# unirestore/UniRestore

Hardware: AMD Instinct MI355X
Metric: restored 512x512 images/sec @ 20 denoise steps (whole job) (higher is better)
Workload: dtype bf16; 1 GPU; PIR 512x512 batch=8/GPU, 20 DDIM steps, bf16, hipGraph replay (BASELINE.json configs[1]; configs[2] shape for N=8); global_batch=8, per_gpu_batch=8, image=512, denoise_steps=20, parallelism=image-parallel dp1, weights=seeded random init (no checkpoints reachable)

## Files before the change

### include/unirestore_hip.h

```cpp
#ifndef UNIRESTORE_HIP_H
#define UNIRESTORE_HIP_H

#include <stddef.h>
#include <stdint.h>

#ifdef __cplusplus
extern "C" {
#endif

typedef void* ur_stream_t;

enum { UR_OK = 0, UR_E_INVALID = -1, UR_E_UNSUPPORTED = -2, UR_E_LAUNCH = -3, UR_E_WORKSPACE = -4 };

enum { UR_DT_BF16 = 0, UR_DT_F16 = 1 };

enum {
  UR_ACT_NONE = 0,
  UR_ACT_SILU = 1,
  UR_ACT_GELU = 2,
  UR_ACT_GEGLU = 3,
  UR_ACT_GATE = 4,
  UR_ACT_TANH = 5,
  UR_ACT_RELU = 6
};

int ur_version(void);
const char* ur_last_error(void);

typedef struct ur_conv_desc {
  const void* x;
  const void* x2;
  const void* w;
  const float* bias;
  const void* residual;
  void* y;
  void* yt;
  float* gn_part;
  const float* gn_ab;
  int gn_silu;
  float* row_stats;
  const float* ln_stats;
  const float* ln_colsum;
  float ln_eps;
  int ln_dim;
  int ln_parts;
  float* workspace;
  size_t workspace_bytes;
  int N, H, W;
  int C1, ldx, C2, ldx2;
  int Cout, ldw, ldy, ldr;
  int KH, KW, stride, pad_t, pad_l;
  int OH, OW;
  int upsample2x;
  int act;
  int out_f32;
  int n_split, t_rows, t_ld;
  float out_scale;
  int nbatch;
  long long bs_x, bs_x2, bs_w, bs_bias, bs_y, bs_r;
  int k_chunk_major;
  long long bias_img_stride;
  int dtype;
  const void* w_frag;
} ur_conv_desc;

int ur_conv2d_nhwc(const ur_conv_desc* d, ur_stream_t stream);

typedef struct ur_conv_plan {
  int row_stat_parts;
  int gn_parts;
  int gn_fused;
  int prologue_ok;
} ur_conv_plan;
int ur_conv2d_plan(const ur_conv_desc* d, ur_conv_plan* plan);

typedef struct ur_conv_launch_info {
  int launcher;
  int splitk;
  int nk_per_split;
  int reduce;
  int reduce_ri;
  int gn_pass;
  int group_loop;
} ur_conv_launch_info;
int ur_conv2d_plan_launch(const ur_conv_desc* d, ur_conv_launch_info* info);
int ur_conv_launcher_count(void);
const char* ur_conv_launcher_name(int i);

int ur_gemm_bias_act(const void* x, const void* w, const float* bias, const void* residual, void* y, long long M, int N, int K,
                     int ldx, int ldw, int ldy, int ldr, int act, float* workspace, size_t workspace_bytes, int dtype,
                     ur_stream_t stream);
int ur_groupconv3x3_nhwc(const void* x, const void* w, const float* bias, void* y, int N, int H, int W, int Cg, int Cog,
                         int groups, int act, float* workspace, size_t workspace_bytes, int dtype, ur_stream_t stream);

int ur_groupnorm_stats_parts(int N, int HW, int C);
size_t ur_groupnorm_ws_bytes(int N, int HW, int C);
size_t ur_groupnorm_ab_bytes(int N, int C);
int ur_groupnorm_stats(const void* x, float* part, int N, int HW, int C, int dtype, ur_stream_t stream);
int ur_instnorm_stats(const void* x, float* part, int N, int HW, int C, int dtype, ur_stream_t stream);
int ur_groupnorm_finalize(const float* part1, int parts1, int C1, const float* part2, int parts2, int C2, const float* gamma,
                          const float* beta, int N, int HW, int G, float eps, float* ab, float* mean_out, ur_stream_t stream);
int ur_groupnorm_apply_act(const void* x, const void* x2, void* y, const float* ab, int N, int HW, int C1, int C2, int silu,
                           int dtype, ur_stream_t stream);
int ur_groupnorm_nhwc(const void* x, const void* x2, void* y, const float* gamma, const float* beta, int N, int HW,
                      int C1, int C2, int G, float eps, int silu, float* ws, float* ab, const float* pre1, int parts1,
                      const float* pre2, int parts2, int dtype, ur_stream_t stream);
int ur_layernorm_rows(const void* x, void* y, const float* gamma, const float* beta, long long rows, int C,
                      float eps, int dtype, ur_stream_t stream);
int ur_softmax_rows_f32(const float* s, void* p, long long rows, int cols, int ldp, int dtype, ur_stream_t stream);

int ur_attention_fwd(const void* q, const void* k, const void* vt, void* o, int B, int H, int Tq, int Tk,
                     int D, int ldq, int ldk, int ldvt, int ldo, long long bs_q, long long bs_k,
                     long long bs_vt, long long bs_o, float scale, int dtype, ur_stream_t stream);
size_t ur_attention_workspace_bytes(int B, int H, int Tq, int Tk, int D);
int ur_attention_fwd_ws(const void* q, const void* k, const void* vt, void* o, int B, int H, int Tq, int Tk,
                        int D, int ldq, int ldk, int ldvt, int ldo, long long bs_q, long long bs_k, long long bs_vt,
                        long long bs_o, float scale, void* ws, size_t ws_bytes, int dtype, ur_stream_t stream);
typedef struct ur_attention_plan {
  int kernel;
  int workgroups;
  int n_full;
  int n_split;
} ur_attention_plan;
int ur_attention_plan_launch(const void* q, const void* k, const void* vt, void* o, int B, int H, int Tq, int Tk,
                             int D, int ldq, int ldk, int ldvt, int ldo, long long bs_q, long long bs_k, long long bs_vt,
                             long long bs_o, void* ws, size_t ws_bytes, ur_attention_plan* plan);
int ur_attention_kernel_count(void);
const char* ur_attention_kernel_name(int i);

size_t ur_chain_tile_bytes(void);
int ur_ff_geglu_fused(const void* x, const void* stream_w, size_t stream_bytes, void* y, long long T, int C, int hidden, int ldx,
                      int ldy, float ln_eps, int dtype, ur_stream_t stream);

int ur_transformer_head_fused(const void* x, const float* gn_ab, const void* stream_w, size_t stream_bytes, void* h0, void* q, void* k,
                              void* vt, long long T, int tokens_per_image, int C, float ln_eps, int dtype, ur_stream_t stream);
int ur_transformer_tail_fused(const void* o1, const void* h0, const void* xres, const void* stream_w, size_t stream_bytes, void* y,
                              float* gn_part, long long T, int tokens_per_image, int C, int hidden, int heads, int tk, float ln_eps,
                              float attn_scale, int dtype, ur_stream_t stream);

int ur_csce_fused(const void* x, const void* cond, const void* stream_w, size_t stream_bytes, void* y, float* gn_part, long long T,
                  int tokens_per_image, int C, int Ccond, int dtype, ur_stream_t stream);

int ur_dwconv3x3_nhwc(const void* x, const float* w9c, const float* bias, void* y, int N, int H, int W, int C,
                      int gate, int dtype, ur_stream_t stream);
int ur_avgpool_hw(const void* x, float* out, int N, int HW, int C, float* ws, int dtype, ur_stream_t stream);
int ur_scale_channels(const void* x, const float* s, const void* residual, void* y, int N, int HW, int C,
                      int dtype, ur_stream_t stream);
int ur_axpy_channels(const void* a, const void* b, const float* s, void* y, long long rows, int C, int dtype, ur_stream_t stream);
int ur_spade_modulate(const void* n, const void* gb, int ldgb, const void* residual, void* y, long long rows, int C,
                      int dtype, ur_stream_t stream);
int ur_linear_f32(const float* x, const float* w, const float* bias, float* y, int M, int N, int K, int groups,
                  int act, ur_stream_t stream);
int ur_tfa_prompt_update(const float* pooled, const float* cond, float* upd, int B, int T, int D, ur_stream_t stream);
int ur_scale_channels_fanout(const void* x, const float* s, void* y, int B, int K, int HW, int C, int dtype, ur_stream_t stream);
int ur_tfa_prompt_update_fanout(const float* pooled, const float* cond, float* upd, int B, int K, int T, int D, int cond_per_row,
                                ur_stream_t stream);
int ur_vec_mul_group(const float* a, const float* b, float* out, int N, int C, int G, ur_stream_t stream);

int ur_image_to_nhwc(const float* img, void* y, int N, int C, int H, int W, int Cpad, int dtype, ur_stream_t stream);
int ur_nhwc_to_nchw_f32(const void* x, int x_is_f32, float* out, int N, int C, int H, int W, int ld, float mul,
                        float add, int dtype, ur_stream_t stream);
int ur_nchw_f32_to_nhwc(const float* x, void* y, int N, int C, int H, int W, int Cpad, int dtype, ur_stream_t stream);
int ur_image_resize_pad_nhwc(const float* img, void* y, int N, int C, int H, int W, int RH, int RW, int PH, int PW, int Cpad,
                             float mul, float add, int dtype, ur_stream_t stream);
int ur_image_unpad_resize_nchw(const void* x, int x_is_f32, float* out, int N, int C, int XH, int XW, int ld, int CH, int CW,
                               int OH, int OW, float mul, float add, int quantize, int dtype, ur_stream_t stream);
int ur_image_u8_ingest(const uint8_t* src, long long slot_bytes, const int* geom, void* y, int N, int CH, int CW, int Cpad, float mul,
                       float add, int dtype, ur_stream_t stream);
int ur_image_u8_egress(const void* x, int x_is_f32, uint8_t* dst, long long slot_bytes, const int* geom, int* nonfinite, int N, int C,
                       int XH, int XW, int ld, float mul, float add, int dtype, ur_stream_t stream);
int ur_vae_sample(const float* moments, int ld, const float* noise_nchw, float* z_nhwc, void* z_16, int N,
                  int HW, int Clat, int Cpad, float scale, int dtype, ur_stream_t stream);
int ur_add_noise(const float* z0, const float* noise_nchw, float* zt, void* zt_16, int N, int HW, int Clat,
                 int Cpad, float sa, float sb, int dtype, ur_stream_t stream);
int ur_ddim_step(float* zt, const float* eps, int ld_eps, void* zt_16, long long M, int Clat, int Cpad,
                 float c_x, float c_e, int dtype, ur_stream_t stream);
int ur_latent_tiles_gather(const float* z, void* tiles_16, int N, int LH, int LW, int Cpad, int T, int th, int tw,
                           const int* origins, int dtype, ur_stream_t stream);
int ur_latent_tiles_blend_ddim(float* zt, const float* eps_tiles, int ld_eps, void* zt_tiles_16, const float* wn, int N, int LH,
                               int LW, int Clat, int Cpad, int T, int th, int tw, const int* origins, float c_x, float c_e,
                               int dtype, ur_stream_t stream);
int ur_f32_to_bf16_scaled(const float* x, int ld, void* y, long long M, int C, int Cpad, float mul, int dtype, ur_stream_t stream);

int ur_keyed_noise(const uint32_t* keys, uint32_t draw, void* out, int N, long long count, int kind, ur_stream_t stream);

int ur_image_metrics(const float* pred, const float* target, int N, int C, int H, int W, int win, double data_range,
                     double* psnr, double* ssim, void* ws, long long ws_bytes, ur_stream_t stream);
long long ur_image_metrics_ws_size(int N, int C, int H, int W, int win);

int ur_lpips_prep(const float* x, float* y, int N, int C, int H, int W, ur_stream_t stream);
int ur_conv2d_f32_wpack_dims(int Cin, int Cout, int KH, int KW, int* kpad, int* cout_pad);
int ur_conv2d_f32(const float* x, const float* w, const float* bias, float* y, int N, int H, int W, int Cin, int Cout, int KH, int KW,
                  int stride, int pad, int relu, ur_stream_t stream);
int ur_maxpool2d_f32(const float* x, float* y, int N, int H, int W, int C, ur_stream_t stream);
int ur_lpips_tap_hw(int H, int W, int tap, int* oh, int* ow);
long long ur_lpips_layer_parts(long long P);
int ur_lpips_layer(const float* feat, const float* lin, int N, int P, int C, double* part, long long part_bytes, ur_stream_t stream);
long long ur_lpips_ws_size(int N, int H, int W);
int ur_lpips_finish(const void* ws, long long ws_bytes, int N, int H, int W, double* out, ur_stream_t stream);

int ur_conv2d_f32_res(const float* x, const float* w, const float* bias, const float* res, float* y, int N, int H, int W, int Cin, int Cout,
                      int KH, int KW, int stride, int pad, int relu, ur_stream_t stream);
int ur_classify_preprocess(const float* x, float* tmp, float* y, int N, int C, int H, int W, const int* first_w, const int* count_w,
                           const float* wt_w, int taps_w, const int* first_h, const int* count_h, const float* wt_h, int taps_h,
                           ur_stream_t stream);
int ur_maxpool2d_pad_f32(const float* x, float* y, int N, int H, int W, int C, ur_stream_t stream);
int ur_avgpool_f32(const float* x, float* y, int N, int P, int C, ur_stream_t stream);
int ur_top1_counts(const float* logits, const long long* labels, int N, int C, long long* pred, long long* counts, ur_stream_t stream);

int ur_color_fix_wavelet(const void* c_f32, int ld_c, const void* src_16, int ld_s, float* out, int N, int src_n, int H, int W, int dtype,
                         ur_stream_t stream);
int ur_color_fix_adain(const void* c_f32, int ld_c, const void* src_16, int ld_s, float* out, int N, int src_n, int H, int W, int dtype,
                       void* ws, size_t ws_bytes, ur_stream_t stream);
size_t ur_color_fix_adain_ws_bytes(int N, int H, int W);

int ur_corrupt_noise(const uint8_t* x, const uint32_t* keys, void* out, int N, int H, int W, int mode, float c, const uint32_t* table,
                     int out_kind, ur_stream_t stream);
int ur_corrupt_filter_sep(const uint8_t* x, const float* taps, int radius, void* out, int N, int H, int W, void* ws, size_t ws_bytes,
                          int out_kind, ur_stream_t stream);
size_t ur_corrupt_filter_sep_ws_bytes(int N, int H, int W);
int ur_corrupt_taps(const uint8_t* x, const int32_t* taps, int n_taps, int per_image, int border, void* out, int N, int H, int W,
                    int out_kind, ur_stream_t stream);
int ur_corrupt_zoom(const uint8_t* x, const int32_t* layers, int n_layers, void* out, int N, int H, int W, int out_kind, ur_stream_t stream);
int ur_corrupt_color(const uint8_t* x, void* out, int N, int H, int W, int mode, float a, float b, void* ws, size_t ws_bytes, int out_kind,
                     ur_stream_t stream);
size_t ur_corrupt_color_ws_bytes(int N, int H, int W);
int ur_corrupt_pixelate(const uint8_t* x, void* out, int N, int H, int W, int small_h, int small_w, const int32_t* hbox, const int32_t* vbox,
                        const int32_t* ymap, const int32_t* xmap, void* ws, size_t ws_bytes, int out_kind, ur_stream_t stream);
size_t ur_corrupt_pixelate_ws_bytes(int N, int H, int small_w);
int ur_corrupt_fog(const uint8_t* x, const uint32_t* keys, void* out, int N, int H, int W, float c, double decay, void* ws, size_t ws_bytes,
                   int out_kind, ur_stream_t stream);
size_t ur_corrupt_fog_ws_bytes(int N, int H, int W);

int ur_jpeg_roundtrip(const uint8_t* x, uint8_t* out, int N, int H, int W, int quality, int subsampling, void* ws, size_t ws_bytes,
                      ur_stream_t stream);
size_t ur_jpeg_roundtrip_ws_bytes(int N, int H, int W, int subsampling);

int ur_resize_u8(const uint8_t* x, uint8_t* out, int N, int H, int W, int oh, int ow, const int32_t* xbounds, const int32_t* xweights, int xK,
                 int xp, const int32_t* ybounds, const int32_t* yweights, int yK, int yp, void* ws, size_t ws_bytes, ur_stream_t stream);
size_t ur_resize_u8_ws_bytes(int N, int H, int W, int oh, int ow);

int ur_distort_shuffle(const uint8_t* x, const uint32_t* keys, uint8_t* out, int N, int H, int W, int delta, uint32_t draw, ur_stream_t stream);
int ur_distort_snow_layer(const uint32_t* keys, float* field, int N, int H, int W, int top, int left, int ch, int cw, int oh, int ow, float loc,
                          float scale, float thr, ur_stream_t stream);
int ur_distort_snow(const uint8_t* x, const float* field, const int32_t* taps, int n_taps, void* out, int N, int H, int W, int oh, int ow,
                    float keep, void* ws, size_t ws_bytes, int out_kind, ur_stream_t stream);
size_t ur_distort_snow_ws_bytes(int N, int H, int W);
int ur_distort_field(const uint32_t* keys, const float* taps_y, int ry, const float* taps_x, int rx, float* field, int N, int H, int W, float m,
                     float alpha, void* ws, size_t ws_bytes, ur_stream_t stream);
size_t ur_distort_field_ws_bytes(int N, int H, int W);
int ur_distort_warp(const uint8_t* x, const float* field, void* out, int N, int H, int W, int out_kind, ur_stream_t stream);

int ur_profile_enable(int on);
int ur_profile_report(char* buf, size_t buf_bytes);

#ifdef __cplusplus
// ... 4 lines not shown
```

### unirestore_amd/capi.py

```python
import ctypes as C
import os

import torch

_HERE = os.path.dirname(os.path.abspath(__file__))
LIB_PATH = os.environ.get("UR_LIB") or os.path.join(_HERE, "libunirestore_hip.so")

UR_ACT_NONE, UR_ACT_SILU, UR_ACT_GELU, UR_ACT_GEGLU, UR_ACT_GATE, UR_ACT_TANH, UR_ACT_RELU = range(7)
UR_DT_BF16, UR_DT_F16 = 0, 1
UR_E_INVALID, UR_E_UNSUPPORTED = -1, -2


class ConvDesc(C.Structure):
    _fields_ = [
        ("x", C.c_void_p), ("x2", C.c_void_p), ("w", C.c_void_p), ("bias", C.c_void_p), ("residual", C.c_void_p),
        ("y", C.c_void_p), ("yt", C.c_void_p), ("gn_part", C.c_void_p), ("gn_ab", C.c_void_p), ("gn_silu", C.c_int),
        ("row_stats", C.c_void_p), ("ln_stats", C.c_void_p), ("ln_colsum", C.c_void_p), ("ln_eps", C.c_float), ("ln_dim", C.c_int), ("ln_parts", C.c_int),
        ("workspace", C.c_void_p),
        ("workspace_bytes", C.c_size_t),
        ("N", C.c_int), ("H", C.c_int), ("W", C.c_int),
        ("C1", C.c_int), ("ldx", C.c_int), ("C2", C.c_int), ("ldx2", C.c_int),
        ("Cout", C.c_int), ("ldw", C.c_int), ("ldy", C.c_int), ("ldr", C.c_int),
        ("KH", C.c_int), ("KW", C.c_int), ("stride", C.c_int), ("pad_t", C.c_int), ("pad_l", C.c_int),
        ("OH", C.c_int), ("OW", C.c_int),
        ("upsample2x", C.c_int), ("act", C.c_int), ("out_f32", C.c_int),
        ("n_split", C.c_int), ("t_rows", C.c_int), ("t_ld", C.c_int),
        ("out_scale", C.c_float),
        ("nbatch", C.c_int),
        ("bs_x", C.c_longlong), ("bs_x2", C.c_longlong), ("bs_w", C.c_longlong), ("bs_bias", C.c_longlong),
        ("bs_y", C.c_longlong), ("bs_r", C.c_longlong), ("k_chunk_major", C.c_int), ("bias_img_stride", C.c_longlong),
        ("dtype", C.c_int), ("w_frag", C.c_void_p),
    ]


class ConvPlan(C.Structure):
    _fields_ = [("row_stat_parts", C.c_int), ("gn_parts", C.c_int), ("gn_fused", C.c_int), ("prologue_ok", C.c_int)]


class ConvLaunchInfo(C.Structure):
    _fields_ = [("launcher", C.c_int), ("splitk", C.c_int), ("nk_per_split", C.c_int), ("reduce", C.c_int), ("reduce_ri", C.c_int),
                ("gn_pass", C.c_int), ("group_loop", C.c_int)]


class AttentionPlan(C.Structure):
    _fields_ = [("kernel", C.c_int), ("workgroups", C.c_int), ("n_full", C.c_int), ("n_split", C.c_int)]


_P, _I, _F, _LL, _SZ = C.c_void_p, C.c_int, C.c_float, C.c_longlong, C.c_size_t

SIGNATURES = {
    "ur_version": (_I, []),
    "ur_last_error": (C.c_char_p, []),
    "ur_conv2d_nhwc": (_I, [C.POINTER(ConvDesc), _P]),
    "ur_conv2d_plan": (_I, [C.POINTER(ConvDesc), C.POINTER(ConvPlan)]),
    "ur_conv2d_plan_launch": (_I, [C.POINTER(ConvDesc), C.POINTER(ConvLaunchInfo)]),
    "ur_conv_launcher_count": (_I, []),
    "ur_conv_launcher_name": (C.c_char_p, [_I]),
    "ur_gemm_bias_act": (_I, [_P, _P, _P, _P, _P, _LL, _I, _I, _I, _I, _I, _I, _I, _P, _SZ, _I, _P]),
    "ur_groupconv3x3_nhwc": (_I, [_P, _P, _P, _P, _I, _I, _I, _I, _I, _I, _I, _P, _SZ, _I, _P]),
    "ur_groupnorm_stats_parts": (_I, [_I, _I, _I]),
    "ur_groupnorm_ws_bytes": (_SZ, [_I, _I, _I]),
    "ur_groupnorm_ab_bytes": (_SZ, [_I, _I]),
    "ur_groupnorm_stats": (_I, [_P, _P, _I, _I, _I, _I, _P]),
    "ur_instnorm_stats": (_I, [_P, _P, _I, _I, _I, _I, _P]),
    "ur_groupnorm_finalize": (_I, [_P, _I, _I, _P, _I, _I, _P, _P, _I, _I, _I, _F, _P, _P, _P]),
    "ur_groupnorm_apply_act": (_I, [_P, _P, _P, _P, _I, _I, _I, _I, _I, _I, _P]),
    "ur_groupnorm_nhwc": (_I, [_P, _P, _P, _P, _P, _I, _I, _I, _I, _I, _F, _I, _P, _P, _P, _I, _P, _I, _I, _P]),
    "ur_layernorm_rows": (_I, [_P, _P, _P, _P, _LL, _I, _F, _I, _P]),
    "ur_softmax_rows_f32": (_I, [_P, _P, _LL, _I, _I, _I, _P]),
    "ur_attention_fwd": (_I, [_P, _P, _P, _P, _I, _I, _I, _I, _I, _I, _I, _I, _I, _LL, _LL, _LL, _LL, _F, _I, _P]),
    "ur_attention_workspace_bytes": (_SZ, [_I, _I, _I, _I, _I]),
    "ur_attention_fwd_ws": (_I, [_P, _P, _P, _P, _I, _I, _I, _I, _I, _I, _I, _I, _I, _LL, _LL, _LL, _LL, _F, _P, _SZ, _I, _P]),
    "ur_attention_plan_launch": (_I, [_P, _P, _P, _P, _I, _I, _I, _I, _I, _I, _I, _I, _I, _LL, _LL, _LL, _LL, _P, _SZ, C.POINTER(AttentionPlan)]),
    "ur_attention_kernel_count": (_I, []),
    "ur_attention_kernel_name": (C.c_char_p, [_I]),
    "ur_chain_tile_bytes": (_SZ, []),
    "ur_ff_geglu_fused": (_I, [_P, _P, _SZ, _P, _LL, _I, _I, _I, _I, _F, _I, _P]),
    "ur_transformer_head_fused": (_I, [_P, _P, _P, _SZ, _P, _P, _P, _P, _LL, _I, _I, _F, _I, _P]),
    "ur_transformer_tail_fused": (_I, [_P, _P, _P, _P, _SZ, _P, _P, _LL, _I, _I, _I, _I, _I, _F, _F, _I, _P]),
    "ur_csce_fused": (_I, [_P, _P, _P, _SZ, _P, _P, _LL, _I, _I, _I, _I, _P]),
    "ur_dwconv3x3_nhwc": (_I, [_P, _P, _P, _P, _I, _I, _I, _I, _I, _I, _P]),
    "ur_avgpool_hw": (_I, [_P, _P, _I, _I, _I, _P, _I, _P]),
    "ur_scale_channels": (_I, [_P, _P, _P, _P, _I, _I, _I, _I, _P]),
    "ur_scale_channels_fanout": (_I, [_P, _P, _P, _I, _I, _I, _I, _I, _P]),
    "ur_axpy_channels": (_I, [_P, _P, _P, _P, _LL, _I, _I, _P]),
    "ur_spade_modulate": (_I, [_P, _P, _I, _P, _P, _LL, _I, _I, _P]),
    "ur_linear_f32": (_I, [_P, _P, _P, _P, _I, _I, _I, _I, _I, _P]),
    "ur_tfa_prompt_update": (_I, [_P, _P, _P, _I, _I, _I, _P]),
    "ur_tfa_prompt_update_fanout": (_I, [_P, _P, _P, _I, _I, _I, _I, _I, _P]),
    "ur_vec_mul_group": (_I, [_P, _P, _P, _I, _I, _I, _P]),
    "ur_image_to_nhwc": (_I, [_P, _P, _I, _I, _I, _I, _I, _I, _P]),
    "ur_nhwc_to_nchw_f32": (_I, [_P, _I, _P, _I, _I, _I, _I, _I, _F, _F, _I, _P]),
    "ur_nchw_f32_to_nhwc": (_I, [_P, _P, _I, _I, _I, _I, _I, _I, _P]),
    "ur_image_resize_pad_nhwc": (_I, [_P, _P] + [_I] * 9 + [_F, _F, _I, _P]),
    "ur_image_unpad_resize_nchw": (_I, [_P, _I, _P] + [_I] * 9 + [_F, _F, _I, _I, _P]),
    "ur_image_u8_ingest": (_I, [_P, _LL, _P, _P, _I, _I, _I, _I, _F, _F, _I, _P]),
    "ur_image_u8_egress": (_I, [_P, _I, _P, _LL, _P, _P, _I, _I, _I, _I, _I, _F, _F, _I, _P]),
    "ur_vae_sample": (_I, [_P, _I, _P, _P, _P, _I, _I, _I, _I, _F, _I, _P]),
    "ur_add_noise": (_I, [_P, _P, _P, _P, _I, _I, _I, _I, _F, _F, _I, _P]),
    "ur_ddim_step": (_I, [_P, _P, _I, _P, _LL, _I, _I, _F, _F, _I, _P]),
    "ur_latent_tiles_gather": (_I, [_P, _P, _I, _I, _I, _I, _I, _I, _I, _P, _I, _P]),
    "ur_latent_tiles_blend_ddim": (_I, [_P, _P, _I, _P, _P, _I, _I, _I, _I, _I, _I, _I, _I, _P, _F, _F, _I, _P]),
    "ur_f32_to_bf16_scaled": (_I, [_P, _I, _P, _LL, _I, _I, _F, _I, _P]),
    "ur_keyed_noise": (_I, [_P, C.c_uint32, _P, _I, _LL, _I, _P]),
    "ur_image_metrics": (_I, [_P, _P, _I, _I, _I, _I, _I, C.c_double, _P, _P, _P, _LL, _P]),
    "ur_image_metrics_ws_size": (_LL, [_I, _I, _I, _I, _I]),
    "ur_lpips_prep": (_I, [_P, _P, _I, _I, _I, _I, _P]),
    "ur_conv2d_f32_wpack_dims": (_I, [_I, _I, _I, _I, C.POINTER(_I), C.POINTER(_I)]),
    "ur_conv2d_f32": (_I, [_P, _P, _P, _P] + [_I] * 10 + [_P]),
    "ur_maxpool2d_f32": (_I, [_P, _P, _I, _I, _I, _I, _P]),
    "ur_lpips_tap_hw": (_I, [_I, _I, _I, C.POINTER(_I), C.POINTER(_I)]),
    "ur_lpips_layer_parts": (_LL, [_LL]),
    "ur_lpips_layer": (_I, [_P, _P, _I, _I, _I, _P, _LL, _P]),
    "ur_lpips_ws_size": (_LL, [_I, _I, _I]),
    "ur_lpips_finish": (_I, [_P, _LL, _I, _I, _I, _P, _P]),
    "ur_conv2d_f32_res": (_I, [_P, _P, _P, _P, _P] + [_I] * 10 + [_P]),
    "ur_classify_preprocess": (_I, [_P, _P, _P, _I, _I, _I, _I, _P, _P, _P, _I, _P, _P, _P, _I, _P]),
    "ur_maxpool2d_pad_f32": (_I, [_P, _P, _I, _I, _I, _I, _P]),
    "ur_avgpool_f32": (_I, [_P, _P, _I, _I, _I, _P]),
    "ur_top1_counts": (_I, [_P, _P, _I, _I, _P, _P, _P]),
    "ur_color_fix_wavelet": (_I, [_P, _I, _P, _I, _P, _I, _I, _I, _I, _I, _P]),
    "ur_color_fix_adain": (_I, [_P, _I, _P, _I, _P, _I, _I, _I, _I, _I, _P, _SZ, _P]),
    "ur_color_fix_adain_ws_bytes": (_SZ, [_I, _I, _I]),
    "ur_corrupt_noise": (_I, [_P, _P, _P, _I, _I, _I, _I, _F, _P, _I, _P]),
    "ur_corrupt_filter_sep": (_I, [_P, _P, _I, _P, _I, _I, _I, _P, _SZ, _I, _P]),
    "ur_corrupt_filter_sep_ws_bytes": (_SZ, [_I, _I, _I]),
    "ur_corrupt_taps": (_I, [_P, _P, _I, _I, _I, _P, _I, _I, _I, _I, _P]),
    "ur_corrupt_zoom": (_I, [_P, _P, _I, _P, _I, _I, _I, _I, _P]),
    "ur_corrupt_color": (_I, [_P, _P, _I, _I, _I, _I, _F, _F, _P, _SZ, _I, _P]),
    "ur_corrupt_color_ws_bytes": (_SZ, [_I, _I, _I]),
    "ur_corrupt_pixelate": (_I, [_P, _P, _I, _I, _I, _I, _I, _P, _P, _P, _P, _P, _SZ, _I, _P]),
    "ur_corrupt_pixelate_ws_bytes": (_SZ, [_I, _I, _I]),
    "ur_corrupt_fog": (_I, [_P, _P, _P, _I, _I, _I, _F, C.c_double, _P, _SZ, _I, _P]),
    "ur_corrupt_fog_ws_bytes": (_SZ, [_I, _I, _I]),
    "ur_jpeg_roundtrip": (_I, [_P, _P, _I, _I, _I, _I, _I, _P, _SZ, _P]),
    "ur_jpeg_roundtrip_ws_bytes": (_SZ, [_I, _I, _I, _I]),
    "ur_resize_u8": (_I, [_P, _P, _I, _I, _I, _I, _I, _P, _P, _I, _I, _P, _P, _I, _I, _P, _SZ, _P]),
    "ur_resize_u8_ws_bytes": (_SZ, [_I, _I, _I, _I, _I]),
    "ur_distort_shuffle": (_I, [_P, _P, _P, _I, _I, _I, _I, C.c_uint32, _P]),
    "ur_distort_snow_layer": (_I, [_P, _P, _I, _I, _I, _I, _I, _I, _I, _I, _I, _F, _F, _F, _P]),
    "ur_distort_snow": (_I, [_P, _P, _P, _I, _P, _I, _I, _I, _I, _I, _F, _P, _SZ, _I, _P]),
    "ur_distort_snow_ws_bytes": (_SZ, [_I, _I, _I]),
    "ur_distort_field": (_I, [_P, _P, _I, _P, _I, _P, _I, _I, _I, _F, _F, _P, _SZ, _P]),
    "ur_distort_field_ws_bytes": (_SZ, [_I, _I, _I]),
    "ur_distort_warp": (_I, [_P, _P, _P, _I, _I, _I, _I, _P]),
    "ur_profile_enable": (_I, [_I]),
    "ur_profile_report": (_I, [C.c_char_p, _SZ]),
}


def _load():
    if not os.path.exists(LIB_PATH):
        raise ImportError(
            f"{LIB_PATH} not found: build it with `python -m unirestore_amd.build` (or __graft_entry__.build()). "
            "There is no CPU / eager fallback in the product path.")
    lib = C.CDLL(LIB_PATH)
    for name, (res, args) in SIGNATURES.items():
        fn = getattr(lib, name)
        fn.restype, fn.argtypes = res, args
    return lib


lib = _load()


def launcher_names() -> list:
    return [lib.ur_conv_launcher_name(i).decode() for i in range(lib.ur_conv_launcher_count())]


def plan_launch(d: ConvDesc) -> ConvLaunchInfo:
    info = ConvLaunchInfo()
    check(lib.ur_conv2d_plan_launch(d, info))
    return info


def attention_kernel_names() -> list:
    return [lib.ur_attention_kernel_name(i).decode() for i in range(lib.ur_attention_kernel_count())]


def attention_plan(q, k, vt, o, B, H, Tq, Tk, D, ldq, ldk, ldvt, ldo, bs_q, bs_k, bs_vt, bs_o, ws, ws_bytes) -> AttentionPlan:
    plan = AttentionPlan()
    check(lib.ur_attention_plan_launch(q, k, vt, o, B, H, Tq, Tk, D, ldq, ldk, ldvt, ldo, bs_q, bs_k, bs_vt, bs_o, ws, ws_bytes, plan))
    return plan


class URError(RuntimeError):
    pass


def check(rc: int):
    if rc != 0:
        msg = lib.ur_last_error().decode("utf-8", "replace")
        if rc == UR_E_INVALID:
            raise ValueError(f"unirestore_hip: {msg}")
        if rc == UR_E_UNSUPPORTED:
            raise NotImplementedError(f"unirestore_hip (UR_E_UNSUPPORTED): {msg}")
        raise URError(f"unirestore_hip error {rc}: {msg}")
```

### unirestore_amd/csrc/igemm.hip

```cpp
#include "igemm_impl.h"

namespace urk {
#define UR_DECLARE(name)                                                                                             \
  ConvLaunch name##_bf16(void* k, size_t ws_bytes);                                                                 \
  ConvLaunch name##_f16(void* k, size_t ws_bytes);                                                                  \
  static ConvLaunch name(ConvK& k, size_t ws_bytes) { return (k.f16 ? name##_f16 : name##_bf16)(&k, ws_bytes); }
UR_CONV_LAUNCHERS(UR_DECLARE)
#undef UR_DECLARE
}

namespace {

ConvLaunch dispatch_conv(ConvK& k, bool pair, size_t ws_bytes) {
  if (k.KH == 3 && k.stride == 1 && k.pad_t == 1 && k.pad_l == 1 && k.kcm && k.staged_ok_ && !pair && k.nbatch == 1 &&
      k.OW % 32 == 0 && k.OH % 8 == 0 && k.OH == (k.ups ? 2 * k.H : k.H) && k.OW == (k.ups ? 2 * k.W : k.W) && !k.yt) {
    const bool ok128 = k.Cout % 128 == 0, ok160 = k.Cout % 160 == 0;
    const long long tm8 = (long long)k.N * (k.OH / 8) * (k.OW / 32);
    auto eff = [](long long t) { return t <= 128 ? (double)(t * (256 / t)) / 256.0 : (double)t / (double)(((t + 255) / 256) * 256); };
    const bool use160 = ok160 && (!ok128 || eff(tm8 * (k.Cout / 160)) >= eff(tm8 * (k.Cout / 128)));
    const long long tiles8 = tm8 * (use160 ? k.Cout / 160 : k.Cout / 128);
    if ((ok128 || ok160) && tiles8 >= 64) {
      if (use160) return urk::halo_8x32_160(k, ws_bytes);
      return urk::halo_8x32_128(k, ws_bytes);
    }
  }
  if (k.KH == 3 && k.stride == 1 && k.pad_t == 1 && k.pad_l == 1 && k.kcm && !pair && k.nbatch == 1 && !k.ups && k.C2 == 0 &&
      k.Cout <= 32 && k.OW % 32 == 0 && k.OH % 8 == 0 && k.OH == k.H && k.OW == k.W && !k.yt && !k.gn_part && !k.gn_ab && !k.row_stats && !k.ln_stats &&
      !k.bias_img && (long long)k.N * (k.OH / 8) * (k.OW / 32) >= 128)
    return urk::halo_thin_32(k, ws_bytes);
  const bool himg_ups = k.ups && k.OH == 16 && k.OW == 16 && k.H == 8 && k.W == 8;
  if (k.KH == 3 && k.stride == 1 && k.pad_t == 1 && k.pad_l == 1 && k.kcm && k.staged_ok_ && !pair && k.nbatch == 1 &&
      ((!k.ups && k.OH == k.H && k.OW == k.W) || himg_ups) && !k.yt && k.Cout % 128 == 0 && k.nk >= 36) {
    if (k.wf && k.OH == 8 && k.OW == 8 && k.N <= 16 && k.Cin % 256 == 0 && k.nk >= 72 && k.y && k.ws && !k.gn_ab && !k.row_stats && !k.ln_stats &&
        (long long)(k.nk / 36) * k.M * k.Cout * 4 <= (long long)ws_bytes)
      return urk::wstream_8x8(k, ws_bytes);
    if (k.OH == 16 && k.OW == 16) return urk::himg_16x16(k, ws_bytes);
    if (k.OH == 8 && k.OW == 8 && k.N % 4 == 0) {
      return urk::himg_8x8x4(k, ws_bytes);
    }
  }
  if (k.KH == 1 && k.stride == 1 && !k.ups && k.C2 == 0 && k.staged_ok_ && k.Cout % 256 == 0 && !k.yt && (k.act == UR_ACT_GEGLU || k.act == UR_ACT_GATE) &&
      (long long)((k.M + 255) / 256) * (k.Cout / 256) * k.nbatch >= 200 && (long long)k.M * k.ldx < (1ll << 31) - 256)
  {
    auto fill = [](long long t) { return (double)t / (double)(((t + 255) / 256) * 256); };
    const long long tm = (k.M + 255) / 256;
    if (k.Cout % 320 == 0 && k.nbatch == 1 && !k.bias_img && fill(tm * (k.Cout / 320)) > fill(tm * (k.Cout / 256)))
      return urk::gemm_256x320_pair(k, ws_bytes);
    return urk::gemm_256x256(k, ws_bytes);
  }
  const bool use_v1 = k.KH == 1 && k.nk <= 10;
  const long long blocks128 = (long long)((k.M + 127) / 128) * ((k.Cout + 127) / 128) * k.nbatch;
  const bool g1 = k.KH == 1 && k.stride == 1 && !k.ups && k.C2 == 0 && k.pad_t == 0 && k.pad_l == 0 && k.OH == k.H && k.OW == k.W &&
                  (long long)k.M * k.ldx + k.Ktot < (1ll << 31) - 256;
  auto nosplit = [&](int bm, int bn) { return (long long)((k.M + bm - 1) / bm) * ((k.Cout + bn - 1) / bn) * k.nbatch >= 200 || k.nk < 8 || !k.ws; };
  if (k.KH == 1 && !pair && k.Cout > 64) {
    const long long blocks64 = (long long)((k.M + 63) / 64) * ((k.Cout + 63) / 64) * k.nbatch;
    if (blocks128 < 200 && g1 && blocks64 >= 128 && blocks64 <= 256 && k.nk >= 8 && k.nk <= 48) return urk::g1_64x64_deep(k, ws_bytes);
    if (g1 && blocks128 < 200 && k.nk > 24 && k.nk <= 96 && (long long)((k.M + 127) / 128) * ((k.Cout + 63) / 64) * k.nbatch >= 256)
      return urk::g1_128x64_deep(k, ws_bytes);
    if (blocks128 < 200 && g1 && ((blocks64 >= 128 && k.nk <= 24) || (blocks64 >= 256 && k.nk <= 48))) return urk::g1_64x64(k, ws_bytes);
    if (blocks128 < 200 && k.nk <= 24) return g1 && nosplit(64, 64) ? urk::g1_64x64(k, ws_bytes) : urk::v1_64x64(k, ws_bytes);
    if (use_v1 && blocks128 > 256 && blocks128 < 400 && k.Cout % 128 == 0) return g1 && nosplit(128, 64) ? urk::g1_128x64(k, ws_bytes) : urk::v1_128x64(k, ws_bytes);
  }
  if (use_v1) {
    if (pair) return urk::v1_128x128(k, ws_bytes);
    if (k.Cout <= 32) return urk::v1_256x32(k, ws_bytes);
    if (k.Cout <= 64) return urk::v1_128x64(k, ws_bytes);
    if (k.Cout % 160 == 0 && k.Cout % 128 != 0) return g1 && nosplit(128, 160) ? urk::g1_128x160(k, ws_bytes) : urk::v1_128x160(k, ws_bytes);
    return g1 && nosplit(128, 128) ? urk::g1_128x128(k, ws_bytes) : urk::v1_128x128(k, ws_bytes);
  }
  if (k.Cout <= 32) return urk::v2_256x32(k, ws_bytes);
  if (k.Cout <= 64 && !pair) return urk::v2_128x64(k, ws_bytes);
  const bool n160 = !pair && k.Cout % 160 == 0 && k.Cout % 128 != 0;
  const long long big_tiles = (long long)((k.M + 255) / 256) * ((k.Cout + (n160 ? 159 : 127)) / (n160 ? 160 : 128)) * k.nbatch;
  if (g1 && !pair && big_tiles < 256) {
    const long long t160 = k.Cout % 160 == 0 ? (long long)((k.M + 127) / 128) * (k.Cout / 160) : 0;
    const long long t128 = (long long)((k.M + 127) / 128) * ((k.Cout + 127) / 128);
    auto fill = [](long long t) { return t <= 0 ? 0.0 : (double)t / (double)(((t + 255) / 256) * 256); };
    if (t160 >= 200 && fill(t160) >= fill(t128)) return urk::g1_128x160(k, ws_bytes);
    if (t128 >= 200) return urk::g1_128x128(k, ws_bytes);
  }
  if (big_tiles >= 160) {
    if (n160 && g1) return urk::g1_128x160(k, ws_bytes);
    if (n160) return urk::v2_256x160(k, ws_bytes);
    return urk::v2_256x128(k, ws_bytes);
  }
  if (k.Cout % 160 == 0 && k.Cout % 128 != 0 && !pair) return urk::v1_128x160(k, ws_bytes);
  return urk::v1_128x128(k, ws_bytes);
}

}

static int conv_impl(const ur_conv_desc* d, ur_stream_t stream, ur_conv_plan* plan, ur_conv_launch_info* info = nullptr) {
  UR_REQUIRE(d && d->x && d->w, "null x/w");
  UR_REQUIRE(d->KH == d->KW && (d->KH == 1 || d->KH == 3), "only 1x1 and 3x3 kernels");
  UR_REQUIRE(d->C1 > 0 && d->C1 % 8 == 0 && d->C2 % 8 == 0 && d->ldx % 8 == 0, "Cin/ldx must be multiples of 8");
  UR_REQUIRE(d->C2 == 0 || (d->x2 && d->ldx2 % 8 == 0), "virtual concat needs x2");
  UR_REQUIRE(d->Cout > 0 && d->Cout % 4 == 0 && d->ldw % 8 == 0, "Cout%4, ldw%8");
  UR_REQUIRE(d->nbatch >= 1 && d->stride >= 1 && d->OH > 0 && d->OW > 0, "bad dims");
  UR_REQUIRE(d->y || d->yt || d->gn_part, "no output requested");
  UR_REQUIRE_DT(d->dtype);
  const bool pair = d->act == UR_ACT_GEGLU || d->act == UR_ACT_GATE;
  if (pair && d->Cout % 64 != 0)
    return ur::fail(UR_E_UNSUPPORTED, "ur_conv2d_nhwc: pair activations (GEGLU / SimpleGate) need Cout % 64 == 0 (32-row a|g interleave)");
  UR_REQUIRE(!d->y || (d->out_f32 ? d->ldy % 4 == 0 : d->ldy % 4 == 0), "ldy%4");
  UR_REQUIRE(!d->residual || d->ldr % 4 == 0, "ldr%4");
  UR_REQUIRE(!d->yt || (d->t_rows > 0 && d->n_split % 4 == 0 && !pair), "bad transposed-output spec");

  ConvK k;
  k.x = (const uint16_t*)d->x; k.x2 = (const uint16_t*)d->x2; k.w = (const uint16_t*)d->w; k.bias = d->bias;
  k.res = (const uint16_t*)d->residual; k.y = d->y; k.yt = (uint16_t*)d->yt;
  k.ws = d->workspace;
  k.N = d->N; k.H = d->H; k.W = d->W; k.C1 = d->C1; k.ldx = d->ldx; k.C2 = d->C2; k.ldx2 = d->ldx2;
  k.Cin = d->C1 + d->C2; k.Cout = d->Cout; k.ldw = d->ldw; k.ldy = d->ldy; k.ldr = d->ldr;
  k.KH = d->KH; k.KW = d->KW; k.stride = d->stride; k.pad_t = d->pad_t; k.pad_l = d->pad_l;
  k.OH = d->OH; k.OW = d->OW; k.OHW = d->OH * d->OW; k.ups = d->upsample2x; k.act = d->act; k.out_f32 = d->out_f32;
  k.n_split = d->yt ? d->n_split : d->Cout; k.t_rows = d->t_rows; k.t_ld = d->t_ld;
  k.out_scale = d->out_scale;
  k.M = d->N * d->OH * d->OW; k.Ktot = d->KH * d->KW * k.Cin; k.nk = (k.Ktot + 63) / 64; k.nbatch = d->nbatch;
  k.bs_x = d->bs_x; k.bs_x2 = d->bs_x2; k.bs_w = d->bs_w; k.bs_bias = d->bs_bias; k.bs_y = d->bs_y; k.bs_r = d->bs_r; k.bias_img = d->bias_img_stride;
  UR_REQUIRE(k.M > 0, "empty problem");
  UR_REQUIRE((long long)d->N * d->H * d->W * (long long)std::max(d->ldx, d->ldx2) < (1ll << 31) &&
                 (long long)d->Cout * d->ldw < (1ll << 31), "tensor too large for 32-bit element offsets");

  k.kcm = d->k_chunk_major; k.wf = (const uint16_t*)d->w_frag; k.wmajor = 0; k.xgm = 0; k.xbn = 0; k.patch_tw = 0;
  UR_REQUIRE(!k.kcm || (k.Cin % 64 == 0 && d->C1 % 64 == 0), "k_chunk_major needs C1 and C1+C2 to be multiples of 64");
  k.gn_part = d->gn_part; k.gn_ab = d->gn_ab; k.gn_silu = d->gn_silu; k.f16 = d->dtype == UR_DT_F16; k.gn_fused = 0; k.gn_parts = 0;
  k.ln_parts = d->ln_parts;
  k.row_stats = d->row_stats; k.ln_stats = d->ln_stats; k.ln_colsum = d->ln_colsum; k.ln_eps = d->ln_eps; k.ln_dim = d->ln_dim;
  UR_REQUIRE(!d->ln_stats || (d->ln_colsum && d->ln_dim > 0), "ln_stats needs ln_colsum / ln_dim");
  UR_REQUIRE(!(d->bias_img_stride && (pair || d->ln_stats || d->yt)), "per-image bias rows do not combine with pair activations / LayerNorm folding / transposed columns");
  k.staged_ok_ = (d->y ? (!d->out_f32 && ((d->ldy | d->bs_y) & 7) == 0) : d->gn_part != nullptr) &&
                 (!d->residual || ((d->ldr | d->bs_r) & 7) == 0);
  UR_REQUIRE(!d->gn_part || (!d->out_f32 && !d->yt), "gn_part needs a plain 16-bit output (or none)");
  hipStream_t s = (hipStream_t)stream;
  const double flops = 2.0 * k.M * (double)k.Cout * k.Ktot * k.nbatch;
  const double bytes = 2.0 * ((double)k.M * k.Cin + (double)k.Cout * k.Ktot + (double)k.M * k.Cout) * k.nbatch;
  const char* fam = d->KH == 3 ? "conv3x3_igemm" : "gemm1x1_igemm";
  static const bool prof_shapes = getenv("UR_PROF_SHAPES") != nullptr;
  if (prof_shapes) {
    static std::map<std::string, int> interned;
    char buf[128];
    snprintf(buf, sizeof buf, "%s M%d N%d K%d s%d u%d b%d a%d", d->KH == 3 ? "c3" : "g1", k.M, k.Cout, k.Ktot, d->stride, d->upsample2x,
             k.nbatch, d->act);
    fam = interned.emplace(buf, 0).first->first.c_str();
  }
  const ConvLaunch launch = dispatch_conv(k, pair, d->workspace_bytes);
  const bool group_loop = k.nbatch > 1 && d->KH == 3 && k.kcm && k.stride == 1 && !pair && !k.gn_part && !k.row_stats && !k.ln_stats &&
                          !k.yt && !k.gn_ab && !k.out_f32 && k.staged_ok_ && k.Cout % 128 == 0 && !k.bias_img && k.C2 == 0;
  auto group_k = [&](int b) {
    ConvK kb = k;
    kb.nbatch = 1;
    kb.x = k.x + b * k.bs_x; kb.w = k.w + b * k.bs_w; kb.bias = k.bias ? k.bias + b * k.bs_bias : nullptr;
    kb.res = k.res ? k.res + b * k.bs_r : nullptr;
    kb.y = reinterpret_cast<uint16_t*>(k.y) + b * k.bs_y;
    kb.bs_x = kb.bs_w = kb.bs_bias = kb.bs_y = kb.bs_r = 0;
    return kb;
  };
  if (plan) {
    plan->row_stat_parts = d->row_stats ? (k.splitk > 1 ? 1 : k.tiles_n) : 0;
    plan->gn_parts = k.gn_parts; plan->gn_fused = k.gn_fused; plan->prologue_ok = launch.prologue_ok;
  }
  if (info) {
    ConvK kb = group_loop ? group_k(0) : k;
    const ConvLaunch l = group_loop ? dispatch_conv(kb, pair, d->workspace_bytes) : launch;
    info->launcher = l.id; info->splitk = kb.splitk; info->nk_per_split = kb.nk_per_split;
    const ReducePlan r = kb.splitk > 1 ? plan_splitk_reduce(kb) : ReducePlan{-1, 0};
    info->reduce = r.kind; info->reduce_ri = r.ri;
    info->gn_pass = k.gn_part && !k.gn_fused && !group_loop;
    info->group_loop = group_loop;
  }
  if (plan || info) return UR_OK;
  if (!d->y && d->gn_part && (!k.gn_fused || k.splitk > 1))
    return ur::fail(UR_E_UNSUPPORTED, "ur_conv2d_nhwc: y == NULL needs a launch whose epilogue writes gn_part (see ur_conv2d_plan)");
  if (d->gn_ab && !launch.prologue_ok)
    return ur::fail(UR_E_UNSUPPORTED, "ur_conv2d_nhwc: gn_ab is not supported by this launch (see ur_conv2d_plan.prologue_ok)");
  ur::ProfScope prof(fam, flops, bytes, s);
  UR_REQUIRE(!(d->row_stats || d->ln_stats) || (k.staged_ok_ && k.nbatch == 1 && !d->yt == !d->yt), "row_stats / ln fusion need a bf16 staged output");
  if (group_loop) {
    for (int b = 0; b < d->nbatch; ++b) {
      ConvK kb = group_k(b);
      const int rcb = dispatch_conv(kb, pair, d->workspace_bytes).launch(&kb, s);
      if (rcb != UR_OK) return rcb;
    }
    return UR_OK;
  }
  const int rc = launch.launch(&k, s);
  if (rc != UR_OK) return rc;
  if (k.gn_part && !k.gn_fused) {
    const int ctot = (pair ? k.Cout / 2 : k.Cout) * k.nbatch;
    UR_REQUIRE(k.y && k.ldy == ctot, "gn_part fallback needs a dense output (ldy == channels)");
    return ur::gn_stats_launch(k.y, k.gn_part, k.N, k.OHW, ctot, d->dtype, s);
  }
  return UR_OK;
}

extern "C" int ur_conv2d_nhwc(const ur_conv_desc* d, ur_stream_t stream) { return conv_impl(d, stream, nullptr); }

extern "C" int ur_conv2d_plan(const ur_conv_desc* d, ur_conv_plan* plan) {
  UR_REQUIRE(d && plan, "null pointer");
  ur_conv_desc t = *d;
  if (!t.y && !t.yt && !t.gn_part) t.y = reinterpret_cast<void*>(16);
  return conv_impl(&t, nullptr, plan);
}

extern "C" int ur_conv2d_plan_launch(const ur_conv_desc* d, ur_conv_launch_info* info) {
  UR_REQUIRE(d && info, "null pointer");
  ur_conv_desc t = *d;
  if (!t.y && !t.yt && !t.gn_part) t.y = reinterpret_cast<void*>(16);
  return conv_impl(&t, nullptr, nullptr, info);
}

#define UR_LAUNCHER_NAME(name) #name,
static const char* const kLauncherNames[] = {UR_CONV_LAUNCHERS(UR_LAUNCHER_NAME)};
#undef UR_LAUNCHER_NAME
static_assert(sizeof(kLauncherNames) / sizeof(kLauncherNames[0]) == UR_CONV_LAUNCHER_COUNT, "one name per launcher");

extern "C" int ur_conv_launcher_count(void) { return UR_CONV_LAUNCHER_COUNT; }
extern "C" const char* ur_conv_launcher_name(int i) { return i >= 0 && i < UR_CONV_LAUNCHER_COUNT ? kLauncherNames[i] : nullptr; }

extern "C" int ur_gemm_bias_act(const void* x, const void* w, const float* bias, const void* residual, void* y, long long M, int N, int K,
                                int ldx, int ldw, int ldy, int ldr, int act, float* workspace, size_t workspace_bytes, int dtype,
                                ur_stream_t stream) {
  UR_REQUIRE(M > 0 && M < (1ll << 31), "M out of range");
  ur_conv_desc d = {};
  d.x = x; d.w = w; d.bias = bias; d.residual = residual; d.y = y;
  d.workspace = workspace; d.workspace_bytes = workspace_bytes;
  d.N = 1; d.H = 1; d.W = (int)M; d.C1 = K; d.ldx = ldx; d.Cout = N; d.ldw = ldw; d.ldy = ldy; d.ldr = ldr;
  d.KH = d.KW = 1; d.stride = 1; d.OH = 1; d.OW = (int)M; d.act = act; d.out_scale = 1.f; d.nbatch = 1; d.dtype = dtype;
  return conv_impl(&d, stream, nullptr);
}

extern "C" int ur_groupconv3x3_nhwc(const void* x, const void* w, const float* bias, void* y, int N, int H, int W, int Cg, int Cog,
                                    int groups, int act, float* workspace, size_t workspace_bytes, int dtype, ur_stream_t stream) {
  UR_REQUIRE(groups >= 1 && Cg % 8 == 0 && Cog % 4 == 0, "groups >= 1, Cg % 8 == 0, Cog % 4 == 0");
  ur_conv_desc d = {};
  d.x = x; d.w = w; d.bias = bias; d.y = y;
  d.workspace = workspace; d.workspace_bytes = workspace_bytes;
  d.N = N; d.H = H; d.W = W; d.C1 = Cg; d.ldx = Cg * groups; d.Cout = Cog; d.ldw = 9 * Cg; d.ldy = Cog * groups;
  d.KH = d.KW = 3; d.stride = 1; d.pad_t = d.pad_l = 1; d.OH = H; d.OW = W; d.act = act; d.out_scale = 1.f; d.nbatch = groups;
  d.bs_x = Cg; d.bs_w = (long long)Cog * 9 * Cg; d.bs_bias = Cog; d.bs_y = Cog; d.dtype = dtype;
  return conv_impl(&d, stream, nullptr);
}
```

### unirestore_amd/csrc/igemm_impl.h

```cpp
#pragma once
#include <cstdio>
#include <cstdlib>
#include <map>
#include <string>

#include "common.h"

static __device__ uint4 g_zero_page[8];
typedef uint32_t ig_u32x4 __attribute__((ext_vector_type(4)));

struct ConvLaunch {
  int (*launch)(void* k, hipStream_t s);
  int prologue_ok;
  int id;
};

namespace {

struct ConvK {
  const uint16_t* x; const uint16_t* x2; const uint16_t* w; const float* bias; const uint16_t* res;
  void* y; uint16_t* yt; float* ws; float* gn_part; const float* gn_ab;
  float* row_stats; const float* ln_stats; const float* ln_colsum; float ln_eps; int ln_dim, ln_parts;
  int N, H, W, C1, ldx, C2, ldx2, Cin, Cout, ldw, ldy, ldr, KH, KW, stride, pad_t, pad_l, OH, OW, OHW;
  int ups, act, out_f32, n_split, t_rows, t_ld;
  float out_scale;
  int M, Ktot, nk, tiles_m, tiles_n, splitk, nk_per_split, nbatch;
  long long bs_x, bs_x2, bs_w, bs_bias, bs_y, bs_r, bias_img;
  int gn_fused, gn_parts, gn_silu, f16, staged_ok_;
  int patch_tw;
  int kcm;
  const uint16_t* wf;
  int wmajor;
  int xgm, xbn;
};

__device__ __forceinline__ void xcd_tile_map(const ConvK& p, int id, int& tm, int& tn) {
  const int xcd = id & 7, idx = id >> 3;
  if (p.xgm) {
    const int lm = idx / p.xbn, ln = idx - lm * p.xbn;
    tm = (xcd % p.xgm) * (p.tiles_m / p.xgm) + lm;
    tn = (xcd / p.xgm) * p.xbn + ln;
    return;
  }
  const int nt = p.tiles_m * p.tiles_n, q = nt >> 3, r = nt & 7;
  id = (xcd < r ? xcd * (q + 1) : r * (q + 1) + (xcd - r) * q) + idx;
  if (p.wmajor) { tn = id / p.tiles_m; tm = id - tn * p.tiles_m; }
  else { tm = id / p.tiles_n; tn = id - tm * p.tiles_n; }
}

static inline void pick_xcd_grid(ConvK& k, double W, double A) {
  k.xgm = 0; k.xbn = 0; k.wmajor = 0;
  static const bool off = getenv("UR_NOXCDGRID") != nullptr;
  if (off || k.nbatch != 1) return;
  const long long nt = (long long)k.tiles_m * k.tiles_n;
  double best = 0.9 * (8.0 * W + A);
  if (nt % 8 == 0)
    for (int gm = 4; gm >= 1; gm >>= 1) {
      const int gn = 8 / gm;
      if (k.tiles_m % gm || k.tiles_n % gn) continue;
      const double c = gm * W + gn * A;
      if (c < best) { best = c; k.xgm = gm; k.xbn = k.tiles_n / gn; }
    }
  if (!k.xgm && k.tiles_n >= 8 && W + 8.0 * A < best) k.wmajor = 1;
}

__device__ __forceinline__ bool is_pair_act(int act) { return act == UR_ACT_GEGLU || act == UR_ACT_GATE; }

__device__ __forceinline__ int tile_row_to_m(const ConvK& p, int m0, int r) {
  return p.patch_tw ? m0 + (r / p.patch_tw) * p.OW + (r % p.patch_tw) : m0 + r;
}

template <bool F16>
__device__ __forceinline__ void epi_store(const ConvK& p, int gb, int m, int co, float v[4]) {
  if (p.res) {
    const uint16_t* r = p.res + gb * p.bs_r + (long long)m * p.ldr + co;
    uint2 rv = *reinterpret_cast<const uint2*>(r);
    v[0] += Act<F16>::lo(rv.x); v[1] += Act<F16>::hi(rv.x);
    v[2] += Act<F16>::lo(rv.y); v[3] += Act<F16>::hi(rv.y);
  }
  if (p.yt && co >= p.n_split) {
    int b = m / p.t_rows, t = m - b * p.t_rows;
    int cw = p.Cout - p.n_split;
    uint16_t* o = p.yt + ((long long)b * cw + (co - p.n_split)) * p.t_ld + t;
#pragma unroll
    for (int e = 0; e < 4; ++e) o[(long long)e * p.t_ld] = f2h16<F16>(v[e]);
    return;
  }
  if (!p.y) return;
  if (p.out_f32) {
    float* o = reinterpret_cast<float*>(p.y) + gb * p.bs_y + (long long)m * p.ldy + co;
    *reinterpret_cast<float4*>(o) = make_float4(v[0], v[1], v[2], v[3]);
  } else {
    uint16_t* o = reinterpret_cast<uint16_t*>(p.y) + gb * p.bs_y + (long long)m * p.ldy + co;
    *reinterpret_cast<uint2*>(o) = make_uint2(Act<F16>::pack2(v[0], v[1]), Act<F16>::pack2(v[2], v[3]));
  }
}

__device__ __forceinline__ int epi_act(const ConvK& p, int gb, int m, int co_in, float a[4], const float g[4]) {
  const long long boff = gb * p.bs_bias + (p.bias_img ? (long long)(m / p.OHW) * p.bias_img : 0);
  if (p.bias) {
    const float* b = p.bias + boff + co_in;
    float4 bv = *reinterpret_cast<const float4*>(b);
    a[0] += bv.x; a[1] += bv.y; a[2] += bv.z; a[3] += bv.w;
  }
  int co = co_in;
  if (is_pair_act(p.act)) {
    float gg[4] = {g[0], g[1], g[2], g[3]};
    if (p.bias) {
      float4 bv = *reinterpret_cast<const float4*>(p.bias + boff + co_in + 32);
      gg[0] += bv.x; gg[1] += bv.y; gg[2] += bv.z; gg[3] += bv.w;
    }
#pragma unroll
    for (int e = 0; e < 4; ++e) a[e] *= (p.act == UR_ACT_GEGLU) ? gelu_f(gg[e]) : gg[e];
    co = (co_in >> 6) * 32 + (co_in & 31);
  } else if (p.act != UR_ACT_NONE) {
#pragma unroll
    for (int e = 0; e < 4; ++e) a[e] = apply_act(a[e], p.act);
  }
#pragma unroll
  for (int e = 0; e < 4; ++e) a[e] *= p.out_scale;
  return co;
}

template <int BM, int NC, int NT, int SROW, bool LOAD>
__device__ __forceinline__ void tile_copy(const ConvK& p, uint16_t* g, long long ld, unsigned char* smem, int m0, int M, int c0,
                                          int cmax) {
  constexpr int Q = NC / 8;
  constexpr int TOT = BM * Q, U = 5;
  for (int i0 = threadIdx.x; i0 < TOT; i0 += NT * U) {
    uint4 v[U];
    uint16_t* gp[U];
    uint2* lp[U];
    bool ok[U];
#pragma unroll
    for (int u = 0; u < U; ++u) {
      const int i = i0 + u * NT;
      const int r = i / Q, c = (i - r * Q) * 8;
      const int m = tile_row_to_m(p, m0, i < TOT ? r : 0);
      ok[u] = i < TOT && m < M && c < cmax;
      gp[u] = g + (long long)(ok[u] ? m : m0) * ld + c0 + (ok[u] ? c : 0);
      lp[u] = reinterpret_cast<uint2*>(smem + (ok[u] ? r * SROW + c * 2 : 0));
      if (LOAD) v[u] = *reinterpret_cast<const uint4*>(gp[u]);
      else { const uint2 a = lp[u][0], b = lp[u][1]; v[u] = make_uint4(a.x, a.y, b.x, b.y); }
    }
#pragma unroll
    for (int u = 0; u < U; ++u) {
      if (!ok[u]) continue;
      if (LOAD) { lp[u][0] = make_uint2(v[u].x, v[u].y); lp[u][1] = make_uint2(v[u].z, v[u].w); }
      else {
store16_wt(gp[u], v[u]);
      }
    }
  }
}

template <int FM, int FN, int WTM, int WTN, bool F16>
__device__ __forceinline__ void igemm_epilogue_direct(const ConvK& p, f32x16 (&acc)[FN][FM], int m0, int n0, int wm, int wn,
                                                      int lane, int gb) {
  const int fhalf = lane >> 5, mrow = lane & 31;
  const bool pair = is_pair_act(p.act);
#pragma unroll
  for (int a = 0; a < FN; ++a) {
    if (pair && (a & 1)) continue;
#pragma unroll
    for (int b = 0; b < FM; ++b) {
      int m = tile_row_to_m(p, m0, wm * WTM + b * 32 + mrow);
#pragma unroll
      for (int rg = 0; rg < 4; ++rg) {
        int co_in = n0 + wn * WTN + a * 32 + rg * 8 + fhalf * 4;
        bool ok = m < p.M && co_in < p.Cout;
        float v[4], g[4] = {0.f, 0.f, 0.f, 0.f};
#pragma unroll
        for (int e = 0; e < 4; ++e) v[e] = acc[a][b][rg * 4 + e];
        if (pair) {
          constexpr int a1 = (FN > 1) ? 1 : 0;
#pragma unroll
          for (int e = 0; e < 4; ++e) g[e] = acc[(a + a1) % FN][b][rg * 4 + e];
        }
        int co = co_in;
        if (ok) co = epi_act(p, gb, m, co_in, v, g);
        if (ok) epi_store<F16>(p, gb, m, co, v);
      }
    }
  }
}

template <int FM, int FN, int WTM, int WTN, int BM, int BN, int SROW, int PAIR, int LN, int MULTI, int YT, int ACT, bool F16>
__device__ __forceinline__ void epi_frag_pass(const ConvK& p, f32x16 (&acc)[FN][FM], int m0, int n0, int c0, int wm, int wn, int lane,
                                              int gb, unsigned char* smem, const float* sbias, const float* scol, const float* srow) {
  const int fhalf = lane >> 5, mrow = lane & 31;
  const bool pair_ = PAIR == 2 ? is_pair_act(p.act) : PAIR != 0;
  const bool ln_ = LN == 2 ? p.ln_stats != nullptr : LN != 0;
  const bool multi_ = MULTI == 2 ? (p.bias_img && !p.patch_tw && p.OHW < BM) : MULTI != 0;
  const bool yt_ = YT == 2 ? p.yt != nullptr : YT != 0;
  const bool act_ = ACT == 2 ? p.act != UR_ACT_NONE : ACT != 0;
  const bool has_res = p.res != nullptr;
#pragma unroll
  for (int a = 0; a < FN; ++a) {
    if (pair_ && (a & 1)) continue;
#pragma unroll
    for (int rg = 0; rg < 4; ++rg) {
      const int ln = wn * WTN + a * 32 + rg * 8 + fhalf * 4;
      const int co_in = n0 + ln;
      float4 bv = *reinterpret_cast<const float4*>(sbias + ln);
      float4 gv = make_float4(0.f, 0.f, 0.f, 0.f);
      if (pair_) gv = *reinterpret_cast<const float4*>(sbias + ln + 32);
      const int lco = pair_ ? ((ln >> 6) * 32 + (ln & 31)) : ln;
      const int co = c0 + lco;
      const bool col_ok = co_in < p.Cout;
      float4 sv = make_float4(0.f, 0.f, 0.f, 0.f), sg = make_float4(0.f, 0.f, 0.f, 0.f);
      if (ln_) {
        sv = *reinterpret_cast<const float4*>(scol + ln);
        if (pair_) sg = *reinterpret_cast<const float4*>(scol + ln + 32);
      }
#pragma unroll
      for (int b = 0; b < FM; ++b) {
        const int lm = wm * WTM + b * 32 + mrow;
        if (multi_) {
          const int il = lm / p.OHW;
          bv = *reinterpret_cast<const float4*>(sbias + il * BN + ln);
          if (pair_) gv = *reinterpret_cast<const float4*>(sbias + il * BN + ln + 32);
        }
        float v[4], gq[4] = {0.f, 0.f, 0.f, 0.f};
        constexpr int a1 = (FN > 1) ? 1 : 0;
        if (ln_) {
          const float mean = srow[2 * lm], rstd = srow[2 * lm + 1];
          v[0] = rstd * (acc[a][b][rg * 4] - mean * sv.x) + bv.x;     v[1] = rstd * (acc[a][b][rg * 4 + 1] - mean * sv.y) + bv.y;
          v[2] = rstd * (acc[a][b][rg * 4 + 2] - mean * sv.z) + bv.z; v[3] = rstd * (acc[a][b][rg * 4 + 3] - mean * sv.w) + bv.w;
          if (pair_) {
            gq[0] = rstd * (acc[(a + a1) % FN][b][rg * 4] - mean * sg.x) + gv.x;     gq[1] = rstd * (acc[(a + a1) % FN][b][rg * 4 + 1] - mean * sg.y) + gv.y;
            gq[2] = rstd * (acc[(a + a1) % FN][b][rg * 4 + 2] - mean * sg.z) + gv.z; gq[3] = rstd * (acc[(a + a1) % FN][b][rg * 4 + 3] - mean * sg.w) + gv.w;
          }
        } else {
          v[0] = acc[a][b][rg * 4] + bv.x; v[1] = acc[a][b][rg * 4 + 1] + bv.y;
          v[2] = acc[a][b][rg * 4 + 2] + bv.z; v[3] = acc[a][b][rg * 4 + 3] + bv.w;
          if (pair_) {
            gq[0] = acc[(a + a1) % FN][b][rg * 4] + gv.x; gq[1] = acc[(a + a1) % FN][b][rg * 4 + 1] + gv.y;
            gq[2] = acc[(a + a1) % FN][b][rg * 4 + 2] + gv.z; gq[3] = acc[(a + a1) % FN][b][rg * 4 + 3] + gv.w;
          }
        }
        if (pair_) {
          const float g0 = gq[0], g1 = gq[1], g2 = gq[2], g3 = gq[3];
          if (p.act == UR_ACT_GEGLU) { v[0] *= gelu_f(g0); v[1] *= gelu_f(g1); v[2] *= gelu_f(g2); v[3] *= gelu_f(g3); }
          else { v[0] *= g0; v[1] *= g1; v[2] *= g2; v[3] *= g3; }
        } else if (act_) {
#pragma unroll
          for (int e = 0; e < 4; ++e) v[e] = apply_act(v[e], p.act);
        }
#pragma unroll
        for (int e = 0; e < 4; ++e) v[e] *= p.out_scale;
        const int mg = tile_row_to_m(p, m0, lm);
        const bool ok = col_ok && mg < p.M;
        if (yt_ && co >= p.n_split) {
          if (ok) epi_store<F16>(p, gb, mg, co, v);
          continue;
        }
        uint2* sp = reinterpret_cast<uint2*>(smem + lm * SROW + lco * 2);
        if (has_res) {
          const uint2 rv = *sp;
          v[0] += Act<F16>::lo(rv.x); v[1] += Act<F16>::hi(rv.x);
          v[2] += Act<F16>::lo(rv.y); v[3] += Act<F16>::hi(rv.y);
        }
        if (ok) *sp = make_uint2(Act<F16>::pack2(v[0], v[1]), Act<F16>::pack2(v[2], v[3]));
      }
    }
  }
}

template <int FM, int FN, int WTM, int WTN, int BM, int BN, int NT, int CLS, bool PAIRC, bool F16>
__device__ __forceinline__ void staged_epilogue(const ConvK& p, f32x16 (&acc)[FN][FM], int m0, int n0, int wm, int wn, int lane,
                                                int gb, unsigned char* smem, bool owner, int nimg_tile_in) {
  constexpr int SROW = (PAIRC ? BN : BN * 2) + 8;
  const bool pair = CLS ? is_pair_act(p.act) : false;
  const bool ln = CLS ? p.ln_stats != nullptr : false;
  const bool yt = CLS ? p.yt != nullptr : false;
  const int nimg_tile = CLS ? nimg_tile_in : 1;
  const int c0 = pair ? (n0 >> 1) : n0;
  const int ncols = pair ? BN / 2 : BN;
  const int cmax = min(yt ? p.n_split : (pair ? p.Cout / 2 : p.Cout), c0 + ncols) - c0;
  float* sbias = reinterpret_cast<float*>(smem + BM * SROW);
  float* scol = sbias + 4 * BN;
  float* srow = scol + BN;
  const int img0 = m0 / p.OHW;
  for (int i = threadIdx.x; i < BN * nimg_tile; i += NT) {
    const int il = i / BN, col = i - il * BN;
    const long long boff = gb * p.bs_bias + (p.bias_img ? (long long)min(img0 + il, p.N - 1) * p.bias_img : 0);
    sbias[i] = (p.bias && n0 + col < p.Cout) ? p.bias[boff + n0 + col] : 0.f;
  }
  if (ln) {
    for (int i = threadIdx.x; i < BN; i += NT) scol[i] = n0 + i < p.Cout ? p.ln_colsum[n0 + i] : 0.f;
    for (int r = threadIdx.x; r < BM; r += NT) {
      const int m = min(tile_row_to_m(p, m0, r), p.M - 1);
      float sx = 0.f, sq = 0.f;
// ... 285 lines not shown
    else { cch += 64; while (cch >= p.Cin) { cch -= p.Cin; ++tap; } }
  };
  auto store_tile = [&](int stage) {
    unsigned char* xs = smem + stage * STAGE;
    unsigned char* wsm = xs + BM * 128;
#pragma unroll
    for (int i = 0; i < XP; ++i) {
      int row = i * 32 + lrow;
      *reinterpret_cast<uint4*>(xs + row * 128 + ((chunk ^ ((row >> 1) & 7)) << 4)) = xr[i];
    }
#pragma unroll
    for (int j = 0; j < WP; ++j) {
      int row = j * 32 + lrow;
      *reinterpret_cast<uint4*>(wsm + row * 128 + ((chunk ^ ((row >> 1) & 7)) << 4)) = wr[j];
    }
  };

  f32x16 acc[FN][FM];
#pragma unroll
  for (int a = 0; a < FN; ++a)
#pragma unroll
    for (int b = 0; b < FM; ++b)
#pragma unroll
      for (int e = 0; e < 16; ++e) acc[a][b][e] = 0.f;

  const int frow = lane & 31, fhalf = lane >> 5;
  typedef __attribute__((address_space(3))) void* lptr_t;
  const unsigned kt_x0 = (unsigned)(uintptr_t)(lptr_t)smem + (wm * WTM + frow) * 128 + ((fhalf ^ ((frow >> 1) & 7)) << 4);
  const unsigned kt_w0 = (unsigned)(uintptr_t)(lptr_t)smem + (BM + wn * WTN + frow) * 128 + ((fhalf ^ ((frow >> 1) & 7)) << 4);
  static_assert(WTM % 32 == 0 && ((WTN >> 1) & 7) == 0, "fragment rows must keep the swizzle phase of row 0");
  auto compute = [&](int stage) {
    if constexpr (ktile_gemm_ok<FM, FN>()) {
      unsigned ab[FM];
#pragma unroll
      for (int b = 0; b < FM; ++b) ab[b] = kt_x0 + stage * STAGE + b * 4096;
      ktile_mma<FM, FN, F16>(acc, ab, kt_w0 + stage * STAGE);
      return;
    }
    const unsigned char* xs = smem + stage * STAGE;
    const unsigned char* wsm = xs + BM * 128;
#pragma unroll
    for (int ks = 0; ks < 4; ++ks) {
      const int slot = ks * 2 + fhalf;
      typename Frag<F16>::type bfr[FM], afr[FN];
#pragma unroll
      for (int b = 0; b < FM; ++b) {
        int row = wm * WTM + b * 32 + frow;
        bfr[b] = *reinterpret_cast<const typename Frag<F16>::type*>(xs + row * 128 + ((slot ^ ((row >> 1) & 7)) << 4));
      }
#pragma unroll
      for (int a = 0; a < FN; ++a) {
        int row = wn * WTN + a * 32 + frow;
        afr[a] = *reinterpret_cast<const typename Frag<F16>::type*>(wsm + row * 128 + ((slot ^ ((row >> 1) & 7)) << 4));
      }
#pragma unroll
      for (int a = 0; a < FN; ++a)
#pragma unroll
        for (int b = 0; b < FM; ++b)
          acc[a][b] = mfma16t(afr[a], bfr[b], acc[a][b]);
    }
  };

  if (kt_begin < kt_end) {
    load_tile();
    store_tile(0);
    __syncthreads();
    int stage = 0;
    for (int kt = kt_begin; kt < kt_end; ++kt) {
      const bool more = kt + 1 < kt_end;
      if (more) load_tile();
      compute(stage);
      if (more) store_tile(stage ^ 1);
      __syncthreads();
      stage ^= 1;
    }
  }

  if constexpr (ktile_gemm_ok<FM, FN>()) asm volatile("s_nop 15\n\ts_nop 7" ::: "memory");
  igemm_epilogue<FM, FN, WTM, WTN, BM, BN, 256, F16>(p, acc, m0, n0, wm, wn, lane, gb, sz, smem);
}

template <bool F16>
__global__ __launch_bounds__(256) void splitk_reduce_kernel(const ConvK p) {
  const bool pair = is_pair_act(p.act);
  const int qn = p.Cout / 4;
  long long total = (long long)p.nbatch * p.M * qn;
  for (long long i = blockIdx.x * (long long)blockDim.x + threadIdx.x; i < total; i += (long long)gridDim.x * blockDim.x) {
    int q = (int)(i % qn);
    long long r = i / qn;
    int m = (int)(r % p.M), gb = (int)(r / p.M);
    int co_in = q * 4;
    if (pair && (co_in & 32)) continue;
    float v[4] = {0, 0, 0, 0}, g[4] = {0, 0, 0, 0};
    for (int s = 0; s < p.splitk; ++s) {
      const float* ws = p.ws + ((long long)(s * p.nbatch + gb) * p.M + m) * p.Cout + co_in;
      float4 t = *reinterpret_cast<const float4*>(ws);
      v[0] += t.x; v[1] += t.y; v[2] += t.z; v[3] += t.w;
      if (pair) {
        float4 u = *reinterpret_cast<const float4*>(ws + 32);
        g[0] += u.x; g[1] += u.y; g[2] += u.z; g[3] += u.w;
      }
    }
    int co = epi_act(p, gb, m, co_in, v, g);
    epi_store<F16>(p, gb, m, co, v);
  }
}

template <bool F16>
__global__ __launch_bounds__(256) void splitk_reduce_rows_kernel(const ConvK p) {
  const bool pair = is_pair_act(p.act);
  const int lane = threadIdx.x & 63, wv = threadIdx.x >> 6;
  const int qn = p.Cout / 4;
  for (int m = blockIdx.x * 4 + wv; m < p.M; m += gridDim.x * 4) {
    float mean = 0.f, rstd = 1.f;
    if (p.ln_stats) {
      float sx = 0.f, sq = 0.f;
      for (int q = 0; q < p.ln_parts; ++q) {
        const float2 t2 = *reinterpret_cast<const float2*>(p.ln_stats + 2 * ((long long)q * p.M + m));
        sx += t2.x; sq += t2.y;
      }
      mean = sx / p.ln_dim;
      rstd = rsqrtf(fmaxf(sq / p.ln_dim - mean * mean, 0.f) + p.ln_eps);
    }
    float rsx = 0.f, rsq = 0.f;
    for (int q = lane; q < qn; q += 64) {
      const int co_in = q * 4;
      if (pair && (co_in & 32)) continue;
      float v[4] = {0, 0, 0, 0}, g[4] = {0, 0, 0, 0};
      for (int s = 0; s < p.splitk; ++s) {
        const float* ws = p.ws + ((long long)s * p.M + m) * p.Cout + co_in;
        const float4 t = *reinterpret_cast<const float4*>(ws);
        v[0] += t.x; v[1] += t.y; v[2] += t.z; v[3] += t.w;
        if (pair) {
          const float4 u = *reinterpret_cast<const float4*>(ws + 32);
          g[0] += u.x; g[1] += u.y; g[2] += u.z; g[3] += u.w;
        }
      }
      if (p.ln_stats) {
        const float4 sc = *reinterpret_cast<const float4*>(p.ln_colsum + co_in);
        v[0] = rstd * (v[0] - mean * sc.x); v[1] = rstd * (v[1] - mean * sc.y);
        v[2] = rstd * (v[2] - mean * sc.z); v[3] = rstd * (v[3] - mean * sc.w);
        if (pair) {
          const float4 sg = *reinterpret_cast<const float4*>(p.ln_colsum + co_in + 32);
          g[0] = rstd * (g[0] - mean * sg.x); g[1] = rstd * (g[1] - mean * sg.y);
          g[2] = rstd * (g[2] - mean * sg.z); g[3] = rstd * (g[3] - mean * sg.w);
        }
      }
      const int co = epi_act(p, 0, m, co_in, v, g);
      if (p.yt && co >= p.n_split) {
        epi_store<F16>(p, 0, m, co, v);
        continue;
      }
      if (p.res) {
        const uint2 rv = *reinterpret_cast<const uint2*>(p.res + (long long)m * p.ldr + co);
        v[0] += Act<F16>::lo(rv.x); v[1] += Act<F16>::hi(rv.x);
        v[2] += Act<F16>::lo(rv.y); v[3] += Act<F16>::hi(rv.y);
      }
      const uint2 o = make_uint2(Act<F16>::pack2(v[0], v[1]), Act<F16>::pack2(v[2], v[3]));
      *reinterpret_cast<uint2*>(reinterpret_cast<uint16_t*>(p.y) + (long long)m * p.ldy + co) = o;
      const float a0 = Act<F16>::lo(o.x), a1 = Act<F16>::hi(o.x);
      const float a2 = Act<F16>::lo(o.y), a3 = Act<F16>::hi(o.y);
      rsx += (a0 + a1) + (a2 + a3);
      rsq += (a0 * a0 + a1 * a1) + (a2 * a2 + a3 * a3);
    }
    if (p.row_stats) {
#pragma unroll
      for (int o = 32; o >= 1; o >>= 1) { rsx += __shfl_xor(rsx, o, 64); rsq += __shfl_xor(rsq, o, 64); }
      if (lane == 0) *reinterpret_cast<float2*>(p.row_stats + 2 * (long long)m) = make_float2(rsx, rsq);
    }
  }
}


template <int RI, bool F16>
__global__ __launch_bounds__(256) void splitk_reduce_gn_kernel(const ConvK p) {
  __shared__ float red[16][16][9];
  const int qc = threadIdx.x & 15, rl = threadIdx.x >> 4;
  const int q = blockIdx.x * 16 + qc, qn = p.Cout / 4, co = q * 4;
  const int r0 = blockIdx.y * 16 * RI;
  float sm[4] = {0, 0, 0, 0}, sq[4] = {0, 0, 0, 0};
  if (q < qn) {
    float v[RI][4];
    uint2 rv[RI];
#pragma unroll
    for (int i = 0; i < RI; ++i) {
      const int m = r0 + rl + 16 * i;
#pragma unroll
      for (int e = 0; e < 4; ++e) v[i][e] = 0.f;
      for (int sp = 0; sp < p.splitk; ++sp) {
        const float4 t = *reinterpret_cast<const float4*>(p.ws + ((long long)sp * p.M + m) * p.Cout + co);
        v[i][0] += t.x; v[i][1] += t.y; v[i][2] += t.z; v[i][3] += t.w;
      }
      rv[i] = p.res ? *reinterpret_cast<const uint2*>(p.res + (long long)m * p.ldr + co) : make_uint2(0, 0);
    }
    const float g[4] = {0, 0, 0, 0};
#pragma unroll
    for (int i = 0; i < RI; ++i) {
      const int m = r0 + rl + 16 * i;
      epi_act(p, 0, m, co, v[i], g);
      v[i][0] += Act<F16>::lo(rv[i].x); v[i][1] += Act<F16>::hi(rv[i].x);
      v[i][2] += Act<F16>::lo(rv[i].y); v[i][3] += Act<F16>::hi(rv[i].y);
      const uint2 o = make_uint2(Act<F16>::pack2(v[i][0], v[i][1]), Act<F16>::pack2(v[i][2], v[i][3]));
      store8_wt(reinterpret_cast<uint16_t*>(p.y) + (long long)m * p.ldy + co, o);
      const float a[4] = {Act<F16>::lo(o.x), Act<F16>::hi(o.x), Act<F16>::lo(o.y), Act<F16>::hi(o.y)};
#pragma unroll
      for (int e = 0; e < 4; ++e) { sm[e] += a[e]; sq[e] += a[e] * a[e]; }
    }
  }
#pragma unroll
  for (int e = 0; e < 4; ++e) { red[rl][qc][e] = sm[e]; red[rl][qc][4 + e] = sq[e]; }
  __syncthreads();
  if (threadIdx.x < 128) {
    const int c = threadIdx.x >> 3, e = threadIdx.x & 7;
    const int qq = blockIdx.x * 16 + c;
    if (qq < qn) {
      float a = 0.f;
#pragma unroll
      for (int r = 0; r < 16; ++r) a += red[r][c][e];
      const int img = r0 / p.OHW, pm = (r0 - img * p.OHW) / (16 * RI);
      float* st = p.gn_part + (((long long)img * p.gn_parts + pm) * p.Cout + qq * 4) * 2;
      st[2 * (e & 3) + (e >> 2)] = a;
    }
  }
}

#ifndef UR_TU_F16
#define UR_TU_F16 0
#endif
#if UR_TU_F16
#define URK(name) name##_f16
#else
#define URK(name) name##_bf16
#endif
#define UR_LAUNCHER(name, ...)                                                                                   \
  ConvLaunch URK(name)(void* kp, size_t ws_bytes) {                                                              \
    return {[](void* k, hipStream_t s) { return __VA_ARGS__::launch(*static_cast<ConvK*>(k), s); },              \
            __VA_ARGS__::plan(*static_cast<ConvK*>(kp), ws_bytes), UR_LAUNCHER_##name};                          \
  }
#define UR_CONV_LAUNCHERS(X)                                                                                      \
  X(v1_128x128) X(v1_128x160) X(v1_128x64) X(v1_256x32) X(v1_64x64)                                               \
  X(v2_256x32) X(v2_128x64) X(v2_256x160) X(v2_256x128) X(gemm_256x256) X(gemm_256x320_pair)                      \
  X(g1_128x128) X(g1_128x160) X(g1_128x64) X(g1_64x64) X(g1_64x64_deep) X(g1_128x64_deep)                         \
  X(halo_8x32_160) X(halo_8x32_128) X(halo_thin_32) X(himg_16x16) X(himg_8x8x4) X(wstream_8x8)
#define UR_LAUNCHER_ID(name) UR_LAUNCHER_##name,
enum ConvLauncherId { UR_CONV_LAUNCHERS(UR_LAUNCHER_ID) UR_CONV_LAUNCHER_COUNT };
#undef UR_LAUNCHER_ID
#define UR_F16_SWITCH(k, ...)                  \
  do {                                         \
    constexpr bool F16 = UR_TU_F16 != 0;       \
    __VA_ARGS__;                               \
  } while (0)

struct ReducePlan { int kind, ri; };
static ReducePlan plan_splitk_reduce(const ConvK& k) {
  const bool pair = k.act == UR_ACT_GEGLU || k.act == UR_ACT_GATE;
  if (k.row_stats || k.ln_stats) return {1, 0};
  if (k.gn_part && k.y && !pair && k.staged_ok_ && k.nbatch == 1 && !k.yt && k.OHW % 64 == 0) {
    const long long colb = (k.Cout / 4 + 15) / 16;
    if (colb * (k.M / 64) >= 512) return {2, 4};
    if (colb * (k.M / 32) >= 512) return {2, 2};
    return {2, 1};
  }
  return {0, 0};
}

static void set_gn_plan(ConvK& k, bool direct_ok, int direct_parts) {
  k.gn_fused = 0; k.gn_parts = 0;
  if (!k.gn_part) return;
  if (k.splitk == 1) {
    if (direct_ok) { k.gn_fused = 1; k.gn_parts = direct_parts; }
  } else {
    const ReducePlan r = plan_splitk_reduce(k);
    if (r.kind == 2) { k.gn_fused = 1; k.gn_parts = k.OHW / (16 * r.ri); }
  }
  if (!k.gn_fused) {
    const bool pair = k.act == UR_ACT_GEGLU || k.act == UR_ACT_GATE;
    k.gn_parts = ur::gn_stats_parts(k.N, k.OHW, (pair ? k.Cout / 2 : k.Cout) * k.nbatch);
  }
}

static void plan_splitk(ConvK& k, size_t ws_bytes, long long want, int gran = 1) {
  int splitk = (int)std::max<long long>(want, 1);
  while (splitk > 1 && (long long)splitk * k.nbatch * k.M * k.Cout * 4 > (long long)ws_bytes) --splitk;
  const int units = k.nk / gran, per = (units + splitk - 1) / splitk;
  k.splitk = (units + per - 1) / per;
  k.nk_per_split = per * gran;
}

static void launch_splitk_reduce(ConvK& k, hipStream_t s) {
  const ReducePlan r = plan_splitk_reduce(k);
  if (r.kind == 1) {
    UR_F16_SWITCH(k, hipLaunchKernelGGL(splitk_reduce_rows_kernel<F16>, dim3(std::min((k.M + 3) / 4, 4096)), dim3(256), 0, s, k));
  } else if (r.kind == 2) {
    const long long colb = (k.Cout / 4 + 15) / 16;
    if (r.ri == 4) UR_F16_SWITCH(k, hipLaunchKernelGGL((splitk_reduce_gn_kernel<4, F16>), dim3(colb, k.M / 64), dim3(256), 0, s, k));
    else if (r.ri == 2) UR_F16_SWITCH(k, hipLaunchKernelGGL((splitk_reduce_gn_kernel<2, F16>), dim3(colb, k.M / 32), dim3(256), 0, s, k));
    else UR_F16_SWITCH(k, hipLaunchKernelGGL((splitk_reduce_gn_kernel<1, F16>), dim3(colb, k.M / 16), dim3(256), 0, s, k));
  } else {
    long long total = (long long)k.nbatch * k.M * (k.Cout / 4);
    int rb = (int)std::min<long long>((total + 255) / 256, 2048);
    UR_F16_SWITCH(k, hipLaunchKernelGGL(splitk_reduce_kernel<F16>, dim3(rb), dim3(256), 0, s, k));
  }
}

template <int BM, int BN, int WM, int WN>
struct Cfg {
  static constexpr int lds = 2 * (BM + BN) * 128;
  static_assert(epi_lds_bytes<BM, BN, 256>() <= lds, "epilogue staging must fit the K ring");
  static int plan(ConvK& k, size_t ws_bytes) {
    k.tiles_m = (k.M + BM - 1) / BM;
    k.tiles_n = (k.Cout + BN - 1) / BN;
    const long long blocks = (long long)k.tiles_m * k.tiles_n * k.nbatch;
    long long want = 1;
    if (blocks < 200 && k.nk >= 8 && k.ws && k.y)
      want = std::min<long long>(std::min<long long>((384 + blocks - 1) / blocks, k.nk / 4), 16);
    plan_splitk(k, ws_bytes, want);
    set_gn_plan(k, k.staged_ok_ && BN >= 32 && (k.OHW % BM) == 0, k.OHW / BM);
    return 0;
  }
  static int launch(ConvK& k, hipStream_t s) {
    static ur::DeviceOnce attr_once;
    if (auto once_guard = attr_once.first()) {
      hipFuncSetAttribute(reinterpret_cast<const void*>(&igemm_kernel<BM, BN, WM, WN, false, UR_TU_F16 != 0>), hipFuncAttributeMaxDynamicSharedMemorySize, lds);
      hipFuncSetAttribute(reinterpret_cast<const void*>(&igemm_kernel<BM, BN, WM, WN, true, UR_TU_F16 != 0>), hipFuncAttributeMaxDynamicSharedMemorySize, lds);
    }
    dim3 grid(k.tiles_m * k.tiles_n, k.nbatch, k.splitk);
    pick_xcd_grid(k, (double)k.Cout * k.Ktot, (double)k.N * k.H * k.W * k.Cin);
    const bool g1 = k.KH == 1 && k.stride == 1 && !k.ups && k.C2 == 0 && k.pad_t == 0 && k.pad_l == 0 && k.OH == k.H && k.OW == k.W &&
                    (long long)k.M * k.ldx + k.Ktot < (1ll << 31);
    if (g1) UR_F16_SWITCH(k, hipLaunchKernelGGL((igemm_kernel<BM, BN, WM, WN, true, F16>), grid, dim3(256), lds, s, k));
    else UR_F16_SWITCH(k, hipLaunchKernelGGL((igemm_kernel<BM, BN, WM, WN, false, F16>), grid, dim3(256), lds, s, k));
    if (k.splitk > 1) launch_splitk_reduce(k, s);
    return ur::check_launch("ur_conv2d_nhwc");
  }
};


template <int BM, int BN, int WM, int WN, int NST, bool F16>
__global__ __launch_bounds__(WM* WN * 64) void igemm_glds_kernel(const ConvK p) {
  constexpr int NT = WM * WN * 64, RPP = NT / 8;
  constexpr int WTM = BM / WM, WTN = BN / WN, FM = WTM / 32, FN = WTN / 32;
  constexpr int XP = BM / RPP, WP = (BN + RPP - 1) / RPP, NLD = XP + WP;
  constexpr int STAGE = (BM + BN) * 128;
  static_assert(BM % RPP == 0 && WTM % 32 == 0 && WTN % 32 == 0 && RPP % 16 == 0, "tile/wave shape");
  static_assert(BN % RPP == 0 || (BN % RPP) * 2 == RPP, "partial W pass must be exactly half a pass");
  extern __shared__ __attribute__((aligned(16))) unsigned char smem[];
// ... 1312 lines not shown
```

### unirestore_amd/csrc/norms.hip

```cpp
#include <cstdio>
#include <cstdlib>
#include <map>
#include <string>
#include "common.h"

namespace {

template <bool F16>
__global__ __launch_bounds__(256) void gn_stats_kernel(const uint16_t* __restrict__ x, float* __restrict__ part,
                                                       int HW, int C, int pix_per_block, int CVS) {
  __shared__ float lds[256 * 16];
  const int n = blockIdx.y, t = threadIdx.x, P = gridDim.x;
  const int CV = C >> 3, R = 256 / CVS;
  const int r = t / CVS, vl = t - r * CVS, v = blockIdx.z * CVS + vl;
  const int p_begin = blockIdx.x * pix_per_block, p_end = min(HW, p_begin + pix_per_block);
  float s[8] = {0, 0, 0, 0, 0, 0, 0, 0}, q[8] = {0, 0, 0, 0, 0, 0, 0, 0};
  if (r < R && v < CV) {
    const uint16_t* xi = x + (long long)n * HW * C + v * 8;
    for (int p = p_begin + r; p < p_end; p += 4 * R) {
      uint4 raw[4];
#pragma unroll
      for (int u = 0; u < 4; ++u) {
        const int pp = min(p + u * R, p_end - 1);
        raw[u] = *reinterpret_cast<const uint4*>(xi + (long long)pp * C);
      }
#pragma unroll
      for (int u = 0; u < 4; ++u) {
        if (p + u * R >= p_end) break;
        float f[8];
        unpack8t<F16>(raw[u], f);
#pragma unroll
        for (int e = 0; e < 8; ++e) { s[e] += f[e]; q[e] += f[e] * f[e]; }
      }
    }
  }
  if (r < R) {
#pragma unroll
    for (int e = 0; e < 8; ++e) { lds[(r * 2) * CVS * 8 + vl * 8 + e] = s[e]; lds[(r * 2 + 1) * CVS * 8 + vl * 8 + e] = q[e]; }
  }
  __syncthreads();
  for (int i = t; i < CVS * 8; i += 256) {
    const int c = blockIdx.z * CVS * 8 + i;
    if (c >= C) continue;
    float a = 0.f, b = 0.f;
    for (int rr = 0; rr < R; ++rr) { a += lds[(rr * 2) * CVS * 8 + i]; b += lds[(rr * 2 + 1) * CVS * 8 + i]; }
    *reinterpret_cast<float2*>(part + (((long long)n * P + blockIdx.x) * C + c) * 2) = make_float2(a, b);
  }
}

__global__ void gn_finalize_kernel(const float* __restrict__ p1, int P1, int C1, const float* __restrict__ p2, int P2, int C2,
                                   const float* __restrict__ gamma, const float* __restrict__ beta, int G, float eps,
                                   double inv_cnt, float* __restrict__ ab, float* __restrict__ mean_out) {
  __shared__ double red[2][256];
  const int g = blockIdx.x, n = blockIdx.y, t = threadIdx.x, NT = blockDim.x;
  const int C = C1 + C2, cpg = C / G, c_lo = g * cpg, Pmax = max(P1, P2);
  float ga0 = 1.f, be0 = 0.f;
  if (ab && t < cpg) { ga0 = gamma ? gamma[c_lo + t] : 1.f; be0 = beta ? beta[c_lo + t] : 0.f; }
  double s = 0.0, q = 0.0;
  for (int idx = t; idx < cpg * Pmax; idx += NT) {
    const int p = idx / cpg, c = c_lo + (idx - p * cpg);
    const bool first = c < C1;
    const int P = first ? P1 : P2;
    if (p < P) {
      const float* src = first ? p1 + (((long long)n * P1 + p) * C1 + c) * 2 : p2 + (((long long)n * P2 + p) * C2 + (c - C1)) * 2;
      const float2 v = *reinterpret_cast<const float2*>(src);
      s += (double)v.x; q += (double)v.y;
    }
  }
  if (NT == 64) {
#pragma unroll
    for (int o = 32; o > 0; o >>= 1) { s += __shfl_xor(s, o, 64); q += __shfl_xor(q, o, 64); }
  } else {
    red[0][t] = s; red[1][t] = q;
    __syncthreads();
    for (int o = NT >> 1; o > 0; o >>= 1) {
      if (t < o) { red[0][t] += red[0][t + o]; red[1][t] += red[1][t + o]; }
      __syncthreads();
    }
  }
  const double S = NT == 64 ? s : red[0][0], Q = NT == 64 ? q : red[1][0];
  const double mean = S * inv_cnt;
  const double var = fma(Q, inv_cnt, -mean * mean);
  const float rstd = rsqrtf(fmaxf((float)var, 0.f) + eps);
  if (mean_out && t == 0) mean_out[(long long)n * G + g] = (float)mean;
  if (ab)
    for (int i = t; i < cpg; i += NT) {
      const int c = c_lo + i;
      const float a = rstd * (i == t ? ga0 : (gamma ? gamma[c] : 1.f));
      ab[((long long)n * 2) * C + c] = a;
      ab[((long long)n * 2 + 1) * C + c] = (i == t ? be0 : (beta ? beta[c] : 0.f)) - (float)mean * a;
    }
}

template <bool F16>
__device__ __forceinline__ void gn_apply_body(const uint16_t* __restrict__ x, uint16_t* __restrict__ y,
                                              const float* __restrict__ ab, int HW, int C, int silu,
                                              int pix_per_block, int c_off, int C_total, int CVS, int bx, int bz) {
  const int n = blockIdx.y, t = threadIdx.x;
  const int CV = C >> 3, R = 256 / CVS;
  const int r = t / CVS, v = bz * CVS + (t - r * CVS);
  if (r >= R || v >= CV) return;
  const int p_begin = bx * pix_per_block, p_end = min(HW, p_begin + pix_per_block);
  const uint16_t* xi = x + (long long)n * HW * C + v * 8;
  uint4 raw[4];
  if (p_begin + r < p_end) {
#pragma unroll
    for (int u = 0; u < 4; ++u) raw[u] = *reinterpret_cast<const uint4*>(xi + (long long)min(p_begin + r + u * R, p_end - 1) * C);
  }
  const float* abn = ab + (long long)n * C_total * 2 + c_off + v * 8;
  float a[8], b[8];
#pragma unroll
  for (int e = 0; e < 8; ++e) { a[e] = abn[e]; b[e] = abn[C_total + e]; }
  uint16_t* yo = y + (long long)n * HW * C_total + c_off + v * 8;
  for (int p = p_begin + r; p < p_end; p += 4 * R) {
    if (p != p_begin + r) {
#pragma unroll
      for (int u = 0; u < 4; ++u) {
        const int pp = min(p + u * R, p_end - 1);
        raw[u] = *reinterpret_cast<const uint4*>(xi + (long long)pp * C);
      }
    }
#pragma unroll
    for (int u = 0; u < 4; ++u) {
      const int pp = p + u * R;
      if (pp >= p_end) break;
      float f[8];
      unpack8t<F16>(raw[u], f);
#pragma unroll
      for (int e = 0; e < 8; ++e) {
        float o = f[e] * a[e] + b[e];
        f[e] = silu ? silu_f(o) : o;
      }
      store16_wt(yo + (long long)pp * C_total, pack8t<F16>(f));
    }
  }
}
template <bool F16>
__global__ __launch_bounds__(256) void gn_apply_kernel(const uint16_t* __restrict__ x, uint16_t* __restrict__ y,
                                                       const float* __restrict__ ab, int HW, int C, int silu,
                                                       int pix_per_block, int c_off, int C_total, int CVS) {
  gn_apply_body<F16>(x, y, ab, HW, C, silu, pix_per_block, c_off, C_total, CVS, blockIdx.x, blockIdx.z);
}
template <bool F16>
__global__ __launch_bounds__(256) void gn_apply2_kernel(const uint16_t* __restrict__ x1, const uint16_t* __restrict__ x2, uint16_t* __restrict__ y,
                                                        const float* __restrict__ ab, int HW, int C1, int C2, int silu, int ppb1, int ppb2,
                                                        int cvs1, int cvs2, int slabs1, int chunks1, int chunks2) {
  if ((int)blockIdx.z < slabs1) {
    if ((int)blockIdx.x < chunks1) gn_apply_body<F16>(x1, y, ab, HW, C1, silu, ppb1, 0, C1 + C2, cvs1, blockIdx.x, blockIdx.z);
  } else if ((int)blockIdx.x < chunks2) {
    gn_apply_body<F16>(x2, y, ab, HW, C2, silu, ppb2, C1, C1 + C2, cvs2, blockIdx.x, blockIdx.z - slabs1);
  }
}

template <int VPL, int R, bool F16>
__global__ __launch_bounds__(256) void ln_rows_kernel(const uint16_t* __restrict__ x, uint16_t* __restrict__ y,
                                                      const float* __restrict__ gamma, const float* __restrict__ beta,
                                                      long long rows, int C, float eps) {
  const int lane = threadIdx.x & 63;
  const long long row0 = ((long long)blockIdx.x * 4 + (threadIdx.x >> 6)) * R;
  if (row0 >= rows) return;
  const int CV = C >> 3;
  uint4 raw[R][VPL];
#pragma unroll
  for (int r = 0; r < R; ++r)
#pragma unroll
    for (int j = 0; j < VPL; ++j) {
      const int v = lane + j * 64;
      const long long row = min(row0 + r, rows - 1);
      raw[r][j] = (v < CV) ? *reinterpret_cast<const uint4*>(x + row * C + v * 8) : make_uint4(0, 0, 0, 0);
    }
  float ga[VPL][8], be[VPL][8];
#pragma unroll
  for (int j = 0; j < VPL; ++j) {
    const int v = lane + j * 64;
#pragma unroll
    for (int e = 0; e < 8; ++e) {
      ga[j][e] = (gamma && v < CV) ? gamma[v * 8 + e] : 1.f;
      be[j][e] = (beta && v < CV) ? beta[v * 8 + e] : 0.f;
    }
  }
#pragma unroll
  for (int r = 0; r < R; ++r) {
    if (row0 + r >= rows) break;
    float f[VPL][8];
    float s = 0.f;
#pragma unroll
    for (int j = 0; j < VPL; ++j) {
      unpack8t<F16>(raw[r][j], f[j]);
#pragma unroll
      for (int e = 0; e < 8; ++e) s += f[j][e];
    }
    const float mean = wave_sum(s) / C;
    float q = 0.f;
#pragma unroll
    for (int j = 0; j < VPL; ++j)
      if (lane + j * 64 < CV) {
#pragma unroll
        for (int e = 0; e < 8; ++e) { float d = f[j][e] - mean; q += d * d; }
      }
    const float rstd = rsqrtf(wave_sum(q) / C + eps);
#pragma unroll
    for (int j = 0; j < VPL; ++j) {
      const int v = lane + j * 64;
      if (v < CV) {
        float o[8];
#pragma unroll
        for (int e = 0; e < 8; ++e) o[e] = (f[j][e] - mean) * rstd * ga[j][e] + be[j][e];
        *reinterpret_cast<uint4*>(y + (row0 + r) * C + v * 8) = pack8t<F16>(o);
      }
    }
  }
}

template <bool F16>
__global__ __launch_bounds__(256) void softmax_rows_kernel(const float* __restrict__ s, uint16_t* __restrict__ p, int cols,
                                                           int ldp) {
  __shared__ float red[8];
  const long long row = blockIdx.x;
  const float* sr = s + row * cols;
  const int t = threadIdx.x, lane = t & 63, w = t >> 6;
  float m = -INFINITY;
  for (int i = t; i < cols; i += 256) m = fmaxf(m, sr[i]);
  m = wave_max(m);
  if (lane == 0) red[w] = m;
  __syncthreads();
  m = fmaxf(fmaxf(red[0], red[1]), fmaxf(red[2], red[3]));
  float l = 0.f;
  for (int i = t; i < cols; i += 256) l += __expf(sr[i] - m);
  l = wave_sum(l);
  if (lane == 0) red[4 + w] = l;
  __syncthreads();
  const float inv = 1.f / (red[4] + red[5] + red[6] + red[7]);
  uint16_t* pr = p + row * ldp;
  for (int i = t; i < cols; i += 256) pr[i] = f2h16<F16>(__expf(sr[i] - m) * inv);
  for (int i = cols + t; i < ldp; i += 256) pr[i] = 0;
}

}

static void gn_geom(int N, int HW, int C, int ppt, int& cvs, int& slabs, int& chunks, int& ppb) {
  const int cv = C / 8;
  cvs = cv < 32 ? cv : 32;
  while (cv % cvs) --cvs;
  slabs = cv / cvs;
  const int R = 256 / cvs;
  const long long want = std::max<long long>(1, 2048 / ((long long)N * slabs));
  chunks = (int)std::min<long long>(want, std::max(1, HW / ((HW <= 64 ? std::min(ppt, 2) : ppt) * R)));
  ppb = (HW + chunks - 1) / chunks;
  chunks = (HW + ppb - 1) / ppb;
}

namespace ur {
int gn_stats_parts(int N, int HW, int C) {
  int cvs, slabs, chunks, ppb;
  gn_geom(N, HW, C, 8, cvs, slabs, chunks, ppb);
  return chunks;
}
int gn_stats_launch(const void* x, float* part, int N, int HW, int C, int dtype, hipStream_t s) {
  int cvs, slabs, chunks, ppb;
  gn_geom(N, HW, C, 8, cvs, slabs, chunks, ppb);
  UR_DT_SWITCH(dtype, hipLaunchKernelGGL(gn_stats_kernel<F16>, dim3(chunks, N, slabs), dim3(256), 0, s, (const uint16_t*)x, part, HW, C, ppb, cvs));
  return check_launch("gn_stats");
}
}

extern "C" {

int ur_groupnorm_stats_parts(int N, int HW, int C) { return (N > 0 && HW > 0 && C > 0 && C % 8 == 0) ? ur::gn_stats_parts(N, HW, C) : UR_E_INVALID; }
size_t ur_groupnorm_ws_bytes(int N, int HW, int C) { return (size_t)N * (size_t)std::max(ur_groupnorm_stats_parts(N, HW, C), 1) * C * 2 * sizeof(float); }
size_t ur_groupnorm_ab_bytes(int N, int C) { return (size_t)N * C * 2 * sizeof(float); }

int ur_groupnorm_stats(const void* x, float* part, int N, int HW, int C, int dtype, ur_stream_t stream) {
  UR_REQUIRE(x && part && N > 0 && HW > 0 && C > 0 && C % 8 == 0, "bad args");
  UR_REQUIRE_DT(dtype);
  hipStream_t s = (hipStream_t)stream;
  ur::ProfScope prof("groupnorm_stats", 0.0, 2.0 * N * HW * (double)C, s);
  return ur::gn_stats_launch(x, part, N, HW, C, dtype, s);
}
int ur_instnorm_stats(const void* x, float* part, int N, int HW, int C, int dtype, ur_stream_t stream) {
  return ur_groupnorm_stats(x, part, N, HW, C, dtype, stream);
}

int ur_groupnorm_finalize(const float* part1, int parts1, int C1, const float* part2, int parts2, int C2, const float* gamma,
                          const float* beta, int N, int HW, int G, float eps, float* ab, float* mean_out, ur_stream_t stream) {
  const int C = C1 + (part2 ? C2 : 0);
  UR_REQUIRE(part1 && parts1 > 0 && C1 > 0 && (!part2 || (parts2 > 0 && C2 > 0)), "bad partial planes");
  UR_REQUIRE(G > 0 && C % G == 0 && N > 0 && HW > 0 && (ab || mean_out), "bad args");
  hipStream_t s = (hipStream_t)stream;
  const int cpg = C / G;
  const long long entries = (long long)cpg * std::max(parts1, part2 ? parts2 : 0);
  ur::ProfScope prof("groupnorm_finalize", 0.0, 8.0 * N * ((double)parts1 * C1 + (part2 ? (double)parts2 * C2 : 0.0)), s);
  const int nt = entries <= 1024 ? 64 : 256;
  hipLaunchKernelGGL(gn_finalize_kernel, dim3(G, N), dim3(nt), 0, s, part1, parts1, C1, part2, part2 ? parts2 : 0, part2 ? C2 : 0, gamma, beta, G,
                     eps, 1.0 / ((double)cpg * HW), ab, mean_out);
  return ur::check_launch("ur_groupnorm_finalize");
}

int ur_groupnorm_apply_act(const void* x, const void* x2, void* y, const float* ab, int N, int HW, int C1, int C2, int silu,
                           int dtype, ur_stream_t stream) {
  UR_REQUIRE(x && y && ab && N > 0 && HW > 0, "null pointer / empty");
  UR_REQUIRE_DT(dtype);
  UR_REQUIRE(C1 > 0 && C1 % 8 == 0 && (!x2 || (C2 > 0 && C2 % 8 == 0)), "C1 (and C2 with x2) must be positive multiples of 8");
  const int C = C1 + (x2 ? C2 : 0);
  hipStream_t s = (hipStream_t)stream;
  const char* fam = "groupnorm";
  static const bool prof_shapes = getenv("UR_PROF_SHAPES") != nullptr;
  if (prof_shapes) {
    static std::map<std::string, int> interned;
    char buf[96];
    snprintf(buf, sizeof buf, "gn N%d HW%d C%d+%d", N, HW, C1, x2 ? C2 : 0);
    fam = interned.emplace(buf, 0).first->first.c_str();
  }
  ur::ProfScope prof(fam, 0.0, 4.0 * N * HW * (double)C, s);
  const uint16_t* src[2] = {(const uint16_t*)x, (const uint16_t*)x2};
  const int cs[2] = {C1, x2 ? C2 : 0}, off[2] = {0, C1};
  constexpr int ppt = 2;
  if (cs[1] > 0) {
    int cvs1, slabs1, chunks1, ppb1, cvs2, slabs2, chunks2, ppb2;
    gn_geom(N, HW, cs[0], ppt, cvs1, slabs1, chunks1, ppb1);
    gn_geom(N, HW, cs[1], ppt, cvs2, slabs2, chunks2, ppb2);
    UR_DT_SWITCH(dtype, hipLaunchKernelGGL(gn_apply2_kernel<F16>, dim3(std::max(chunks1, chunks2), N, slabs1 + slabs2), dim3(256), 0, s, src[0], src[1],
                                           (uint16_t*)y, ab, HW, cs[0], cs[1], silu, ppb1, ppb2, cvs1, cvs2, slabs1, chunks1, chunks2));
    return ur::check_launch("ur_groupnorm_apply_act");
  }
  for (int i = 0; i < 2; ++i) {
    if (cs[i] <= 0) continue;
    int cvs, slabs, chunks, ppb;
    gn_geom(N, HW, cs[i], ppt, cvs, slabs, chunks, ppb);
    UR_DT_SWITCH(dtype, hipLaunchKernelGGL(gn_apply_kernel<F16>, dim3(chunks, N, slabs), dim3(256), 0, s, src[i], (uint16_t*)y, ab, HW, cs[i], silu,
                                           ppb, off[i], C, cvs));
  }
  return ur::check_launch("ur_groupnorm_apply_act");
}

int ur_groupnorm_nhwc(const void* x, const void* x2, void* y, const float* gamma, const float* beta, int N, int HW,
                      int C1, int C2, int G, float eps, int silu, float* ws, float* ab, const float* pre1, int parts1,
                      const float* pre2, int parts2, int dtype, ur_stream_t stream) {
  UR_REQUIRE(x && y && ab, "null pointer");
  UR_REQUIRE_DT(dtype);
  UR_REQUIRE(N > 0 && HW > 0 && C1 > 0 && C1 % 8 == 0 && (!x2 || (C2 > 0 && C2 % 8 == 0)), "N, HW, C1 (and C2 with x2) must be positive, C % 8 == 0");
  UR_REQUIRE(G > 0 && (C1 + (x2 ? C2 : 0)) % G == 0, "G must be positive and divide C1 + C2");
  UR_REQUIRE((!pre1 || parts1 > 0) && (!x2 || !pre2 || parts2 > 0), "producer-side partial planes need parts > 0");
  UR_REQUIRE((pre1 && (!x2 || pre2)) || ws, "a source without producer-side partials needs the ws scratch");
  if (!pre1) {
    parts1 = ur::gn_stats_parts(N, HW, C1);
    int rc = ur_groupnorm_stats(x, ws, N, HW, C1, dtype, stream);
    if (rc != UR_OK) return rc;
    pre1 = ws;
    ws += (size_t)N * parts1 * C1 * 2;
  }
  if (x2 && !pre2) {
    parts2 = ur::gn_stats_parts(N, HW, C2);
    int rc = ur_groupnorm_stats(x2, ws, N, HW, C2, dtype, stream);
    if (rc != UR_OK) return rc;
    pre2 = ws;
  }
  int rc = ur_groupnorm_finalize(pre1, parts1, C1, x2 ? pre2 : nullptr, parts2, C2, gamma, beta, N, HW, G, eps, ab, nullptr, stream);
  if (rc != UR_OK) return rc;
  return ur_groupnorm_apply_act(x, x2, y, ab, N, HW, C1, C2, silu, dtype, stream);
}

int ur_avgpool_hw(const void* x, float* out, int N, int HW, int C, float* ws, int dtype, ur_stream_t stream) {
  UR_REQUIRE(x && out && ws && N > 0 && HW > 0 && C > 0 && C % 8 == 0, "bad args");
  UR_REQUIRE_DT(dtype);
  int rc = ur_groupnorm_stats(x, ws, N, HW, C, dtype, stream);
  if (rc != UR_OK) return rc;
  return ur_groupnorm_finalize(ws, ur::gn_stats_parts(N, HW, C), C, nullptr, 0, 0, nullptr, nullptr, N, HW, C, 0.f, nullptr, out, stream);
}

int ur_layernorm_rows(const void* x, void* y, const float* gamma, const float* beta, long long rows, int C, float eps,
                      int dtype, ur_stream_t stream) {
  UR_REQUIRE(x && y && rows > 0, "null pointer / empty");
  UR_REQUIRE(C > 0 && C % 8 == 0 && C <= 2048, "C%8 and 0<C<=2048");
  UR_REQUIRE_DT(dtype);
  hipStream_t s = (hipStream_t)stream;
  ur::ProfScope prof("layernorm", 0.0, 4.0 * rows * (double)C, s);
  const int vpl = (C / 8 + 63) / 64;
  constexpr int R = 4;
  dim3 grid((unsigned)((rows + 4 * R - 1) / (4 * R))), block(256);
  const uint16_t* xi = (const uint16_t*)x;
  uint16_t* yo = (uint16_t*)y;
  switch (vpl) {
    case 1: UR_DT_SWITCH(dtype, hipLaunchKernelGGL((ln_rows_kernel<1, R, F16>), grid, block, 0, s, xi, yo, gamma, beta, rows, C, eps)); break;
    case 2: UR_DT_SWITCH(dtype, hipLaunchKernelGGL((ln_rows_kernel<2, R, F16>), grid, block, 0, s, xi, yo, gamma, beta, rows, C, eps)); break;
    case 3: UR_DT_SWITCH(dtype, hipLaunchKernelGGL((ln_rows_kernel<3, R, F16>), grid, block, 0, s, xi, yo, gamma, beta, rows, C, eps)); break;
    default: UR_DT_SWITCH(dtype, hipLaunchKernelGGL((ln_rows_kernel<4, R, F16>), grid, block, 0, s, xi, yo, gamma, beta, rows, C, eps)); break;
  }
  return ur::check_launch("ur_layernorm_rows");
}

int ur_softmax_rows_f32(const float* sm, void* p, long long rows, int cols, int ldp, int dtype, ur_stream_t stream) {
  UR_REQUIRE(sm && p && rows > 0 && cols > 0 && ldp >= cols, "bad args");
  UR_REQUIRE_DT(dtype);
  hipStream_t s = (hipStream_t)stream;
  ur::ProfScope prof("softmax_rows", 0.0, rows * (double)cols * 6.0, s);
  UR_DT_SWITCH(dtype, hipLaunchKernelGGL(softmax_rows_kernel<F16>, dim3((unsigned)rows), dim3(256), 0, s, sm, (uint16_t*)p, cols, ldp));
  return ur::check_launch("ur_softmax_rows_f32");
}

}
```

### unirestore_amd/csrc/runtime.hip

```cpp
#include <cstring>
#include <mutex>
#include <sstream>
#include <vector>
#include <map>

#include "common.h"

namespace {
__global__ void zero_kernel(uint32_t* p, size_t n) {
  for (size_t i = blockIdx.x * (size_t)blockDim.x + threadIdx.x; i < n; i += (size_t)gridDim.x * blockDim.x) p[i] = 0u;
}
}

namespace ur {

void zero_async(void* ptr, size_t bytes, hipStream_t s) {
  const size_t n = bytes / 4;
  if (n == 0) return;
  const unsigned blocks = (unsigned)std::min<size_t>((n + 255) / 256, 1024);
  hipLaunchKernelGGL(zero_kernel, dim3(blocks), dim3(256), 0, s, (uint32_t*)ptr, n);
}

static thread_local std::string g_err;

void set_error(const std::string& msg) { g_err = msg; }
int fail(int code, const std::string& msg) {
  g_err = msg;
  return code;
}
int check_launch(const char* what) {
  hipError_t e = hipGetLastError();
  if (e != hipSuccess) return fail(UR_E_LAUNCH, std::string(what) + ": " + hipGetErrorString(e));
  return UR_OK;
}

struct ProfRec {
  const char* family;
  double flops, bytes;
  hipEvent_t a, b;
};
static std::mutex g_mu;
static bool g_prof_on = false;
static std::vector<ProfRec> g_recs;
static std::vector<hipEvent_t> g_pool;

static hipEvent_t get_event() {
  if (!g_pool.empty()) {
    hipEvent_t e = g_pool.back();
    g_pool.pop_back();
    return e;
  }
  hipEvent_t e;
  hipEventCreate(&e);
  return e;
}

ProfScope::ProfScope(const char* family, double flops, double bytes, hipStream_t s) : slot(-1), stream(s) {
  if (!g_prof_on) return;
  hipStreamCaptureStatus st = hipStreamCaptureStatusNone;
  if (hipStreamIsCapturing(s, &st) != hipSuccess || st != hipStreamCaptureStatusNone) return;
  std::lock_guard<std::mutex> lk(g_mu);
  ProfRec r{family, flops, bytes, get_event(), get_event()};
  hipEventRecord(r.a, s);
  g_recs.push_back(r);
  slot = (int)g_recs.size() - 1;
}
ProfScope::~ProfScope() {
  if (slot < 0) return;
  std::lock_guard<std::mutex> lk(g_mu);
  hipEventRecord(g_recs[slot].b, stream);
}

}

extern "C" {

int ur_version(void) { return 101; }
const char* ur_last_error(void) { return ur::g_err.c_str(); }

int ur_profile_enable(int on) {
  std::lock_guard<std::mutex> lk(ur::g_mu);
  ur::g_prof_on = on != 0;
  if (on) {
    for (auto& r : ur::g_recs) {
      ur::g_pool.push_back(r.a);
      ur::g_pool.push_back(r.b);
    }
    ur::g_recs.clear();
  }
  return UR_OK;
}

int ur_profile_report(char* buf, size_t buf_bytes) {
  std::lock_guard<std::mutex> lk(ur::g_mu);
  struct Agg { long n = 0; double ms = 0, flops = 0, bytes = 0; };
  std::map<std::string, Agg> agg;
  for (auto& r : ur::g_recs) {
    hipEventSynchronize(r.b);
    float ms = 0.f;
    hipEventElapsedTime(&ms, r.a, r.b);
    Agg& a = agg[r.family];
    a.n++; a.ms += ms; a.flops += r.flops; a.bytes += r.bytes;
  }
  std::ostringstream os;
  os << "{";
  bool first = true;
  for (auto& kv : agg) {
    if (!first) os << ", ";
    first = false;
    os << "\"" << kv.first << "\": {\"launches\": " << kv.second.n << ", \"ms\": " << kv.second.ms
       << ", \"flops\": " << kv.second.flops << ", \"bytes\": " << kv.second.bytes << "}";
  }
  os << "}";
  std::string s = os.str();
  if (s.size() + 1 > buf_bytes) return ur::fail(UR_E_INVALID, "ur_profile_report: buffer too small");
  memcpy(buf, s.c_str(), s.size() + 1);
  return UR_OK;
}

}
```

### unirestore_amd/modules/model.py

```python
import os
import weakref
from typing import Optional

import numpy as np
import torch
import torch.nn as nn
import torch.nn.functional as F

from .. import ops, schedule, tiling
from .adapters import SPADE, CSCEAdapter, TaskFeatureAdapter, cfrm_blocks
from . import nn as nnmod
from .nn import (DEV, AutoencoderKL, Conv2d, DownBlock, MidBlock, ResnetBlock2D, TimestepEmbedding, UNet2DConditionModel,
                 invalidate_packed, sinusoid_table)

stablesr_config = dict(in_channels=4, model_channels=256, out_channels=256, num_res_blocks=2, dropout=0,
                       channel_mult=(1, 1, 2, 2), downsample_type="conv", num_heads=4,
                       down_block_types=("AttnDownBlock2D",) * 3 + ("DownBlock2D",), mid_block_type="UNetMidBlock2D")


TILE_CONTROLLER_MAX_IMAGES = 400


def _use_dtype(module):
    owner = module.__dict__.get("_ur_owner")
    owner = owner() if owner is not None else None
    if owner is not None and owner.__dict__.get("_stale"):
        owner.refresh()
    dt = module.__dict__.get("_ur_dtype")
    if dt is not None:
        ops.set_dtype(dt)


def _check_fp16(*tensors):
    if ops.act_dtype() != torch.float16:
        return
    for t in tensors:
        for v in (t.values() if isinstance(t, dict) else (t,)):
            if not bool(torch.isfinite(v).all()):
                raise FloatingPointError("fp16 activation overflow (|x| > 65504): the result is not finite.  Use dtype='bf16' for these weights")


def _per_sample_timesteps(timesteps, batch):
    ts = [int(t) for t in torch.as_tensor(timesteps).reshape(-1).tolist()]
    if len(ts) != 1 and len(ts) != batch:
        raise ValueError(f"timesteps must hold 1 or {batch} values, got {len(ts)}")
    return ts[:1] if len(set(ts)) == 1 else ts


def _resnets(module):
    return [m for m in module.modules() if isinstance(m, ResnetBlock2D) and m.time_emb_proj is not None]


class Controller(nn.Module):
    def __init__(self, in_channels, model_channels, out_channels, num_res_blocks, dropout, channel_mult,
                 downsample_type, num_heads, down_block_types, mid_block_type, groups=32):
        super().__init__()
        if mid_block_type != "UNetMidBlock2D":
            raise NotImplementedError(mid_block_type)
        self.model_channels = model_channels
        temb = model_channels * 4
        self.time_embedding = TimestepEmbedding(model_channels, temb)
        self.conv_in = Conv2d(in_channels, model_channels, 3, padding=1)
        self.down_blocks = nn.ModuleList()
        chans, out = [], model_channels
        for i, kind in enumerate(down_block_types):
            cin, out = out, model_channels * channel_mult[i]
            last = i == len(channel_mult) - 1
            self.down_blocks.append(DownBlock(cin, out, temb, attn="self" if kind == "AttnDownBlock2D" else None,
                                              head_dim=out // num_heads, add_downsample=not last,
                                              layers=num_res_blocks, groups=groups, eps=1e-5))
            chans.append(out)
        self.middle_block = MidBlock(out, temb, "self", head_dim=out // num_heads, groups=groups, eps=1e-5)
        self.fea_tran = nn.ModuleList([ResnetBlock2D(c, out_channels, temb, groups, 1e-5) for c in chans])
        for m in self.modules():
            if isinstance(m, ResnetBlock2D):
                nn.init.zeros_(m.conv2.weight), nn.init.zeros_(m.conv2.bias)
            if hasattr(m, "to_out") and hasattr(m, "group_norm"):
                nn.init.zeros_(m.to_out[0].weight), nn.init.zeros_(m.to_out[0].bias)

    def set_timesteps(self, timesteps):
        emb = self.time_embedding.silu_emb(sinusoid_table(timesteps, self.model_channels))
        for r in _resnets(self):
            r.set_time_table(emb)
        self.table_epoch = getattr(self, "table_epoch", 0) + 1

    def stem(self, z_bf16):
        return ops.conv(z_bf16, self.conv_in.packed(), gn=True)

    def run(self, stem, step):
        feats, h = [], stem
        for blk in self.down_blocks:
            states = []
            for i, res in enumerate(blk.resnets):
                h = res.run(h, step=step)
                if blk.attn_kind == "self":
                    h = blk.attentions[i].run(h)
                states.append(h)
            if blk.downsamplers is not None:
                h = blk.downsamplers[0].run(h)
                states.append(h)
            feats.append(states[-2])
        feats[-1] = self.middle_block.run(h, step=step)
        return {f.shape[2]: self.fea_tran[i].run(f, step=step) for i, f in enumerate(feats)}

    def run_schedule(self, stem, nsteps):
        b = stem.shape[0]
        x = stem.repeat(nsteps, 1, 1, 1)
        g = ops.gn_of(stem)
        if g is not None:
            x._gn = (g[0].repeat(nsteps, 1, 1, 1), g[1])
        out = self.run(x, "all")
        return [{k: v[i * b:(i + 1) * b] for k, v in out.items()} for i in range(nsteps)]

    def run_steps(self, stem, s0, s1):
        b, n = stem.shape[0], s1 - s0
        x = stem.repeat(n, 1, 1, 1)
        g = ops.gn_of(stem)
        if g is not None:
            x._gn = (g[0].repeat(n, 1, 1, 1), g[1])
        out = self.run(x, slice(s0, s1))
        return [{k: v[i * b:(i + 1) * b] for k, v in out.items()} for i in range(n)]

    def forward(self, x, timesteps, encoder_hidden_states=None):
        _use_dtype(self)
        ts = _per_sample_timesteps(timesteps, x.shape[0])
        self.set_timesteps(ts)
        out = self.run(self.stem(ops.nchw_to_nhwc(x.to(DEV))), 0 if len(ts) == 1 else "all")
        out = {k: ops.nhwc_to_nchw(v) for k, v in out.items()}
        _check_fp16(out)
        return out


class ControlledUNet(nn.Module):
    def __init__(self, unet: UNet2DConditionModel, control_type: str, null_embeds: Optional[torch.Tensor] = None,
                 cond_channels: int = 256):
        super().__init__()
        self.unet = unet
        cross_dim = unet.down_blocks[0].attentions[0].transformer_blocks[0].attn2.to_k.in_features
        if null_embeds is None:
            p = os.path.join(os.path.dirname(os.path.abspath(__file__)), "..", "assets", "sd_null_emb.pt")
            null_embeds = torch.load(p, map_location="cpu") if (cross_dim == 1024 and os.path.exists(p)) else \
                torch.zeros(1, 77, cross_dim)
        self.register_buffer("null_embeds", null_embeds.float())
        self.control_type = control_type
        if control_type == "spade":
            for m in list(unet.modules()):
                if isinstance(m, ResnetBlock2D):
                    m.spade = SPADE(m.conv2.out_channels, cond_channels)
        elif control_type == "scedit":
            chans = [unet.conv_in.out_channels]
            for blk in unet.down_blocks:
                chans += [r.conv2.out_channels for r in blk.resnets]
                if blk.downsamplers is not None:
                    chans.append(chans[-1])
            self.csc_editors = nn.ModuleList([CSCEAdapter(c, c, cond_channels) for c in chans])
        else:
            raise ValueError(f"control_type '{control_type}' not supported")

    def set_timesteps(self, timesteps):
        u = self.unet
        emb = u.time_embedding.silu_emb(sinusoid_table(timesteps, u.time_proj_dim))
        for r in _resnets(u):
            r.set_time_table(emb)
        self.table_epoch = getattr(self, "table_epoch", 0) + 1

    def _ctx(self):
        key = ("ctx", ops.act_dtype())
        if key not in self.__dict__:
            self.__dict__[key] = self.null_embeds.to(DEV, ops.act_dtype()).contiguous()
        return self.__dict__[key]

    def run(self, zt_bf16, control, step):
        u, ctx = self.unet, self._ctx()
        h = ops.conv(zt_bf16, u.conv_in.packed(), gn=True)
        skips = [h]
        sp = control if self.control_type == "spade" else None
        for blk in u.down_blocks:
            for i, res in enumerate(blk.resnets):
                h = res.run(h, step=step, control=sp)
                if blk.attn_kind == "cross":
                    h = blk.attentions[i].run(h, ctx)
                skips.append(h)
            if blk.downsamplers is not None:
                h = blk.downsamplers[0].run(h)
                skips.append(h)
        raw = skips
        if sp is not None:
            h = u.mid_block.run(h, step=step, ctx=ctx, control=sp)
            edited = raw
        else:
            h = u.mid_block.run(h, step=step, ctx=ctx)
            edited = [ed.run(s, control[s.shape[2]]) for ed, s in zip(self.csc_editors, raw)]
        idx = len(raw)
        for blk in u.up_blocks:
            for i, res in enumerate(blk.resnets):
                idx -= 1
                h = res.run(h, x2=edited[idx], step=step, control=sp)
                if blk.attn_kind == "cross":
                    h = blk.attentions[i].run(h, ctx)
            if blk.upsamplers is not None:
                h = blk.upsamplers[0].run(h)
        h = u.conv_norm_out.run(h, silu=True)
        return ops.conv(h, u.conv_out.packed(), out_f32=True)

    def forward(self, sample, control, timesteps):
        _use_dtype(self)
        ts = _per_sample_timesteps(timesteps, sample.shape[0])
        self.set_timesteps(ts)
        ctl = {k: ops.nchw_to_nhwc(v.to(DEV)) for k, v in control.items()}
        eps = self.run(ops.nchw_to_nhwc(sample.to(DEV)), ctl, 0 if len(ts) == 1 else "all")
        eps = ops.nhwc_to_nchw(eps, c=self.unet.conv_out.out_channels)
        _check_fp16(eps)
        return eps


class SkipConnectedAutoEncoder(nn.Module):
    def __init__(self, vae: AutoencoderKL, fr_type: Optional[str] = None, tedit: Optional[dict] = None, fr_depths=(1, 1, 9)):
        super().__init__()
        self.tedit_dict = tedit
        self.vae = vae
        enc_ch = [b.resnets[-1].conv2.out_channels for b in vae.encoder.down_blocks]
        if fr_type == "CFRM":
            vae.encoder.fr_blocks = cfrm_blocks(enc_ch[:3], fr_depths)
        elif fr_type is not None:
            raise ValueError("Invalid fr_type")
        if tedit:
            self.task_list = list(tedit["task"])
            self.tedit_type = tedit["type"]
            if self.tedit_type != "TFA":
                raise KeyError("%s is not defined in the taskeditor!, please select ['TFA']" % self.tedit_type)
            pl, top = tedit["prompt_len"], enc_ch[-1]
            vae.decoder.task_prompts = nn.ParameterDict({t: nn.Parameter(torch.zeros(pl, enc_ch[2])) for t in self.task_list})
            vae.decoder.task_editors = nn.ModuleList([
                TaskFeatureAdapter(top, enc_ch[2], prompt_len=pl),
                TaskFeatureAdapter(top, enc_ch[1], prompt_len=pl),
                TaskFeatureAdapter(top, enc_ch[0], prompt_len=pl, last_layer=True)])
        else:
            self.task_list, self.tedit_type = [], None

    def encode_run(self, images_dev: torch.Tensor, noise_nchw: torch.Tensor, enable_fr: bool, plan=None, return_input=False):
        enc, lat = self.vae.encoder, self.vae.latent_channels
        if isinstance(plan, RaggedIO):
            x0 = plan.ingest(images_dev)
        else:
            x0 = ops.image_resize_pad(images_dev, *plan) if plan else ops.nchw_to_nhwc(images_dev, image=True)
        h = ops.conv(x0, enc.conv_in.packed(), gn=True)
        res = []
        for i, blk in enumerate(enc.down_blocks[:-1]):
            h = blk.run(h)
            if enable_fr:
                h = enc.fr_blocks[i].run(h)
            res.append(h)
        h = enc.mid_block.run(enc.down_blocks[-1].run(h))
        h = ops.conv(enc.conv_norm_out.run(h, silu=True), enc.conv_out.packed())
        moments = ops.conv(h, self.vae.quant_conv.packed(), out_f32=True)
        z, zb = ops.vae_sample(moments, noise_nchw, lat, self.vae.config.scaling_factor)
        return (z, zb, res, x0) if return_input else (z, zb, res)

    def _egress(self, x, out_plan, color_src=None, color_fix=None):
        c = self.vae.decoder.conv_out.out_channels
        if color_src is not None and color_fix is not None:
            x = ops.color_fix(x, color_src, color_fix)
        if isinstance(out_plan, RaggedIO):
            return out_plan.egress(x, c)
        if out_plan:
            return ops.image_unpad_resize(x, c, out_plan[0], out_plan[1], mul=0.5, add=0.5, quantize=out_plan[2])
        return ops.nhwc_to_nchw(x, c=c, mul=0.5, add=0.5)

    def decode_run(self, z_f32: torch.Tensor, res_samples, task: str, out_plan=None, color_src=None, color_fix=None):
        dec, lat = self.vae.decoder, self.vae.latent_channels
        if self.tedit_dict and task not in dec.task_prompts:
            raise KeyError(task)
        zb = ops.f32_to_bf16(z_f32, lat, mul=1.0 / self.vae.config.scaling_factor)
# ... 525 lines not shown
```

### unirestore_amd/modules/nn.py

```python
import math
from typing import Optional

import os

import torch
import torch.nn as nn

from .. import chain, ops
from ..ops import UR_ACT_GEGLU, UR_ACT_GELU, UR_ACT_NONE, UR_ACT_SILU

DEV = "cuda"
CHAIN = os.environ.get("UR_CHAIN", "1") == "1"


class _NoEager:
    def forward(self, *a, **k):
        raise RuntimeError(f"{type(self).__name__}: no eager/PyTorch path exists; use the HIP-backed graph")


class Conv2d(_NoEager, nn.Conv2d):
    def packed(self, pair=False, scale: Optional[torch.Tensor] = None) -> ops.PackedConv:
        key = ("pk", pair, ops.act_dtype())
        if key not in self.__dict__:
            w, b = self.weight, self.bias
            if scale is not None:
                s = scale.detach().reshape(-1)
                w = w * s[:, None, None, None]
                b = None if b is None else b * s
            self.__dict__[key] = ops.pack_conv(w, b, DEV, pair=pair, groups=self.groups)
        return self.__dict__[key]


class Linear(_NoEager, nn.Linear):
    def packed(self, pair=False) -> ops.PackedConv:
        key = ("pk", pair, ops.act_dtype())
        if key not in self.__dict__:
            self.__dict__[key] = ops.pack_conv(self.weight, self.bias, DEV, pair=pair)
        return self.__dict__[key]

    def dev_f32(self):
        if "f32" not in self.__dict__:
            self.__dict__["f32"] = (self.weight.detach().float().to(DEV).contiguous(),
                                    None if self.bias is None else self.bias.detach().float().to(DEV).contiguous())
        return self.__dict__["f32"]


class _Affine:
    def dev(self):
        if "aff" not in self.__dict__:
            self.__dict__["aff"] = (self.weight.detach().float().to(DEV).contiguous(),
                                    self.bias.detach().float().to(DEV).contiguous())
        return self.__dict__["aff"]


class GroupNorm(_NoEager, _Affine, nn.GroupNorm):
    def run(self, x, silu=False, x2=None):
        g, b = self.dev()
        return ops.group_norm(x, g, b, self.num_groups, self.eps, silu, x2=x2)

    def coeffs(self, x, x2=None):
        g, b = self.dev()
        return ops.gn_finalize(x, g, b, self.num_groups, self.eps, x2=x2)


class LayerNorm(_NoEager, _Affine, nn.LayerNorm):
    def run(self, x):
        g, b = self.dev()
        return ops.layer_norm(x, g, b, self.eps)


def invalidate_packed(model: nn.Module):
    for m in model.modules():
        for k in [k for k in m.__dict__ if k in ("aff", "f32", "dw", "vecs") or
                  (isinstance(k, tuple) and k[0] in ("pk", "cache", "fused", "ctx", "gb"))]:
            del m.__dict__[k]


def sinusoid_table(timesteps, dim: int) -> torch.Tensor:
    half = dim // 2
    freqs = torch.exp(-math.log(10000.0) * torch.arange(half, dtype=torch.float32) / half)
    ang = torch.as_tensor(list(timesteps), dtype=torch.float32).reshape(-1, 1) * freqs.reshape(1, -1)
    return torch.cat([torch.cos(ang), torch.sin(ang)], dim=-1)


class TimestepEmbedding(nn.Module):
    def __init__(self, in_dim, time_dim):
        super().__init__()
        self.linear_1 = Linear(in_dim, time_dim)
        self.linear_2 = Linear(time_dim, time_dim)

    def silu_emb(self, sin_table: torch.Tensor) -> torch.Tensor:
        w1, b1 = self.linear_1.dev_f32()
        w2, b2 = self.linear_2.dev_f32()
        h = ops.linear_f32(sin_table.to(DEV), w1, b1, UR_ACT_SILU)
        return ops.linear_f32(h, w2, b2, UR_ACT_SILU)


class ResnetBlock2D(nn.Module):
    def __init__(self, cin, cout, temb_channels=None, groups=32, eps=1e-5):
        super().__init__()
        self.norm1 = GroupNorm(groups, cin, eps=eps)
        self.conv1 = Conv2d(cin, cout, 3, padding=1)
        self.time_emb_proj = Linear(temb_channels, cout) if temb_channels else None
        self.norm2 = GroupNorm(groups, cout, eps=eps)
        self.conv2 = Conv2d(cout, cout, 3, padding=1)
        self.conv_shortcut = Conv2d(cin, cout, 1) if cin != cout else None
        self.tbias = None

    def set_time_table(self, silu_emb: torch.Tensor):
        for k in [k for k in self.__dict__ if isinstance(k, tuple) and k[:2] == ("cache", "tb_all")]:
            del self.__dict__[k]
        w, b = self.time_emb_proj.dev_f32()
        cb = self.conv1.bias.detach().float().to(DEV)
        self.tbias = ops.linear_f32(silu_emb, w, b + cb)

    def _tbias_all(self, b, steps=None):
        key = ("cache", "tb_all", b) if steps is None else ("cache", "tb_all", b, steps.start, steps.stop)
        if key not in self.__dict__:
            rows = self.tbias if steps is None else self.tbias[steps]
            self.__dict__[key] = rows.repeat_interleave(b, dim=0).contiguous()
        return self.__dict__[key]

    def run(self, x, x2=None, step=None, sample_bias=None, control=None):
        bias = None
        if self.time_emb_proj is not None:
            if sample_bias is not None:
                bias = sample_bias
            elif isinstance(step, str):
                bias = self._tbias_all(x.shape[0] // self.tbias.shape[0])
            elif isinstance(step, slice):
                bias = self._tbias_all(x.shape[0] // (step.stop - step.start), step)
            else:
                bias = self.tbias[step]
        h = gn_silu_conv(self.norm1, x, self.conv1.packed(), x2=x2, bias=bias, gn=True)
        pc2 = self.conv2.packed()
        if self.conv_shortcut is not None:
            sc = ops.conv(x, self.conv_shortcut.packed(), x2=x2)
        else:
            sc = x
        if control is not None and "spade" in self._modules:
            if x2 is not None and self.conv_shortcut is None:
                raise ValueError("identity shortcut cannot take a virtual concat")
            h = gn_silu_conv(self.norm2, h, pc2, gn=True)
            return self.spade.run(h, control[h.shape[2]], residual=sc)
        return gn_silu_conv(self.norm2, h, pc2, residual=sc, gn=True)


FUSE_GN_MIN_PIXELS = 256 * 256
FUSE_GN_MAX_COUT = 256


def gn_silu_conv(norm: "GroupNorm", x, pc, x2=None, **kw):
    ab = norm.coeffs(x, x2=x2)
    if x.shape[1] * x.shape[2] >= FUSE_GN_MIN_PIXELS and pc.cout_out <= FUSE_GN_MAX_COUT and \
            ops.conv_plan(x, pc, x2=x2, gn=kw.get("gn", False), gn_ab=True, residual=kw.get("residual") is not None).prologue_ok:
        return ops.conv(x, pc, x2=x2, gn_ab=ab, gn_silu=True, **kw)
    return ops.conv(ops.gn_apply(x, ab, silu=True, x2=x2), pc, **kw)


class Downsample2D(nn.Module):
    def __init__(self, c, padding):
        super().__init__()
        self.padding = padding
        self.conv = Conv2d(c, c, 3, stride=2, padding=padding)

    def run(self, x):
        n, h, w, _ = x.shape
        if self.padding == 0:
            return ops.conv(x, self.conv.packed(), stride=2, pad=(0, 0), out_hw=(h // 2, w // 2), gn=True)
        return ops.conv(x, self.conv.packed(), stride=2, pad=(1, 1), gn=True)


class Upsample2D(nn.Module):
    def __init__(self, c):
        super().__init__()
        self.conv = Conv2d(c, c, 3, padding=1)

    def run(self, x):
        return ops.conv(x, self.conv.packed(), upsample=True, gn=True)


class _ToOut(nn.ModuleList):
    def __init__(self, c):
        super().__init__([Linear(c, c), nn.Identity()])


Q_FOLD = math.log2(math.e)
LN2 = math.log(2.0)


def _scaled_first(ts, q_scale):
    ts = [None if t is None else t.detach().float() for t in ts]
    if q_scale != 1.0 and ts[0] is not None:
        ts[0] = ts[0] * q_scale
    return ts


def _fused_qkv(mod, names, q_scale=1.0):
    ck = ("cache", "qkv", ops.act_dtype(), q_scale)
    if ck not in mod.__dict__:
        ws = _scaled_first([getattr(mod, n).weight for n in names], q_scale)
        bs = _scaled_first([getattr(mod, n).bias for n in names], q_scale)
        mod.__dict__[ck] = ops.pack_conv(torch.cat(ws, 0), None if bs[0] is None else torch.cat(bs, 0), DEV)
    return mod.__dict__[ck]


def _fused_ln(mod, key, names, norm, pair=False, q_scale=1.0):
    ck = ("cache", "ln", key, ops.act_dtype(), q_scale)
    if ck not in mod.__dict__:
        ws = _scaled_first([getattr(mod, n).weight for n in names], q_scale)
        bs = _scaled_first([getattr(mod, n).bias for n in names], q_scale)
        mod.__dict__[ck] = ops.pack_linear_ln(torch.cat(ws, 0), None if bs[0] is None else torch.cat(bs, 0), norm.weight, norm.bias, norm.eps,
                                               DEV, pair=pair)
    return mod.__dict__[ck]


def self_attention(mod, h, heads, residual, gn_kw={}, ln=None, rows=False):
    b, t, c = h.shape
    d = c // heads
    ldvt = ops.round_up(t, 8)
    vt = torch.zeros((b, c, ldvt), dtype=h.dtype, device=h.device) if ldvt != t else \
        torch.empty((b, c, ldvt), dtype=h.dtype, device=h.device)
    scale = 1.0 / math.sqrt(d)
    qs = scale * Q_FOLD if d == 64 else 1.0
    if ln is not None:
        qk = ops.linear(h, _fused_ln(mod, "qkv", ("to_q", "to_k", "to_v"), ln[0], q_scale=qs), ln_stats=ln[1], yt=vt, n_split=2 * c, t_rows=t)
    else:
        qk = ops.linear(h, _fused_qkv(mod, ("to_q", "to_k", "to_v"), q_scale=qs), yt=vt, n_split=2 * c, t_rows=t)
    if d in (64, 128, 512):
        o = ops.attention(qk, qk[:, :, c:], vt, heads, d, t, t, LN2 if d == 64 else scale, ldq=3 * c, ldk=3 * c,
                          bs_q=t * 3 * c, bs_k=t * 3 * c, bs_vt=c * ldvt, batch=b)
    else:
        o = attention_gemm(qk[:, :, :c], qk[:, :, c:2 * c], vt, heads, d, t)
    return ops.linear(o, mod.to_out[0].packed(), residual=residual, rows=rows, **gn_kw)


def attention_gemm(q, k, vt, heads, d, t, s_bytes=256 << 20):
    b = q.shape[0]
    rows = max(256, min(t, (s_bytes // (4 * b * t)) // 256 * 256))
    out = torch.empty((b, t, heads * d), dtype=q.dtype, device=q.device)
    for hh in range(heads):
        qh, kh, vh = q[:, :, hh * d:(hh + 1) * d], k[:, :, hh * d:(hh + 1) * d], vt[:, hh * d:(hh + 1) * d, :]
        for r0 in range(0, t, rows):
            r1 = min(t, r0 + rows)
            s = ops.bmm_nt(qh[:, r0:r1], kh, out_f32=True, out_scale=1.0 / math.sqrt(d))
            p = ops.softmax_rows(s, ldp=vt.shape[-1])
            out[:, r0:r1, hh * d:(hh + 1) * d] = ops.bmm_nt(p, vh)
    return out


class AttentionBlock(nn.Module):

    def __init__(self, c, head_dim, groups=32, eps=1e-5):
        super().__init__()
        self.heads = c // head_dim
        self.group_norm = GroupNorm(groups, c, eps=eps)
        self.to_q, self.to_k, self.to_v = Linear(c, c), Linear(c, c), Linear(c, c)
        self.to_out = _ToOut(c)

    def run(self, x):
        n, hh, ww, c = x.shape
        h = self.group_norm.run(x).view(n, hh * ww, c)
        o = self_attention(self, h, self.heads, x.view(n, hh * ww, c), gn_kw=dict(gn=True, gn_hw=(n, hh * ww)))
        return ops.carry(o, o.view(n, hh, ww, c))


class CrossAttention(nn.Module):
    def __init__(self, c, heads, kv_dim=None):
        super().__init__()
        self.heads = heads
        kv_dim = kv_dim or c
        self.to_q = Linear(c, c, bias=False)
        self.to_k = Linear(kv_dim, c, bias=False)
        self.to_v = Linear(kv_dim, c, bias=False)
        self.to_out = _ToOut(c)

    def context_kv(self, ctx: torch.Tensor):
        key = ("cache", "ctx", ops.act_dtype())
        if key not in self.__dict__:
            tk = ctx.shape[1]
            c = self.to_q.out_features
            kv = _fused_qkv(self, ("to_k", "to_v"))
            vt = torch.zeros((1, c, ops.round_up(tk, 8)), dtype=ctx.dtype, device=DEV)
            k = ops.linear(ctx, kv, yt=vt, n_split=c, t_rows=tk)
            self.__dict__[key] = (k, vt, tk)
        return self.__dict__[key]

    def run_cross(self, h, ctx, residual, ln=None, rows=False):
        b, t, c = h.shape
        d = c // self.heads
        k, vt, tk = self.context_kv(ctx)
        if ln is not None:
            q = ops.linear(h, _fused_ln(self, "q", ("to_q",), ln[0]), ln_stats=ln[1])
        else:
            q = ops.linear(h, self.to_q.packed())
        o = ops.attention(q, k, vt, self.heads, d, t, tk, 1.0 / math.sqrt(d), ldq=c, ldk=2 * c, bs_q=t * c, bs_k=0,
                          bs_vt=0, batch=b)
        return ops.linear(o, self.to_out[0].packed(), residual=residual, rows=rows)
# ... 238 lines not shown
```

### unirestore_amd/ops.py

```python
from dataclasses import dataclass
from typing import Optional

import torch

from . import capi
from .capi import (UR_ACT_GATE, UR_ACT_GEGLU, UR_ACT_GELU, UR_ACT_NONE, UR_ACT_RELU, UR_ACT_SILU, UR_ACT_TANH, UR_DT_BF16,
                   UR_DT_F16, ConvDesc, ConvPlan, check, lib)

BF16 = torch.bfloat16
F16 = torch.float16
_ws = {}

_DTYPES = {"bf16": BF16, "bfloat16": BF16, BF16: BF16, "fp16": F16, "float16": F16, "f16": F16, "16": F16, F16: F16}
_act = BF16


def set_dtype(dt) -> torch.dtype:
    global _act
    if dt not in _DTYPES:
        raise ValueError(f"unsupported compute dtype {dt!r}: choose 'bf16' or 'fp16'")
    _act = _DTYPES[dt]
    return _act


def act_dtype() -> torch.dtype:
    return _act


def _dt(t: Optional[torch.Tensor] = None) -> int:
    d = _act if t is None else t.dtype
    if d == BF16:
        return UR_DT_BF16
    if d == F16:
        return UR_DT_F16
    raise TypeError(f"expected a bf16 / fp16 tensor, got {d}")


def _stream():
    return torch.cuda.current_stream().cuda_stream


def _ptr(t: Optional[torch.Tensor]):
    return None if t is None else t.data_ptr()


def workspace(dev, nbytes=192 << 20) -> torch.Tensor:
    key = (dev, "splitk")
    if key not in _ws:
        _ws[key] = torch.empty(nbytes // 4, dtype=torch.float32, device=dev)
    return _ws[key]


def ln_of(t):
    return getattr(t, "_ln", None)


def gn_of(t):
    return getattr(t, "_gn", None)


def carry(src, dst):
    g = getattr(src, "_gn", None)
    if g is not None:
        dst._gn = g
    r = getattr(src, "_ln", None)
    if r is not None:
        dst._ln = r
    return dst


def round_up(v, m):
    return (v + m - 1) // m * m


@dataclass
class PackedConv:
    w: torch.Tensor
    bias: Optional[torch.Tensor]
    cin: int
    cout: int
    cout_out: int
    k: int
    groups: int = 1
    pair: bool = False
    ln_colsum: Optional[torch.Tensor] = None
    ln_eps: float = 0.0
    kcm: bool = False
    w_frag: Optional[torch.Tensor] = None

    def frag(self) -> torch.Tensor:
        if self.w_frag is None:
            nt, nc = self.cout // 128, self.cin // 64
            w = self.w.view(nt, 4, 32, nc, 9, 4, 2, 8)
            self.w_frag = w.permute(0, 3, 4, 5, 1, 6, 2, 7).contiguous()
        return self.w_frag


def wants_frag(pc: "PackedConv", n, h, w_, c1, c2, stride, upsample, groups) -> bool:
    return (pc.k == 3 and pc.kcm and groups == 1 and stride == 1 and not upsample and h == 8 and w_ == 8 and n <= 16 and not pc.pair
            and pc.cout % 128 == 0 and (c1 + c2) % 256 == 0 and (c1 + c2) >= 512 and (c2 == 0 or c1 % 64 == 0))


def pack_conv(weight: torch.Tensor, bias: Optional[torch.Tensor], dev, *, pair=False, groups=1, cin_pad=None, c1=None, group_halo=False) -> PackedConv:
    w = weight.detach().to(dev, torch.float32)
    if w.dim() == 2:
        w = w[:, :, None, None]
    cout, cin_g, kh, kw = w.shape
    assert kh == kw and kh in (1, 3)
    cin_p = cin_pad or round_up(cin_g, 8)
    cout_p = round_up(cout, 8)
    if groups > 1:
        assert cin_g % 8 == 0 and (cout // groups) % 4 == 0
    if cin_p == cin_g and cout_p == cout:
        wp = w.permute(0, 2, 3, 1).contiguous()
    else:
        wp = torch.zeros(cout_p, kh, kw, cin_p, dtype=torch.float32, device=dev)
        wp[:cout, :, :, :cin_g] = w.permute(0, 2, 3, 1)
    b = None
    if bias is not None:
        b = torch.zeros(cout_p, dtype=torch.float32, device=dev)
        b[:cout] = bias.detach().to(dev, torch.float32)
    cout_out = cout_p
    if pair:
        half = cout // 2
        if cout % 2 or half % 32:
            raise NotImplementedError(f"UR_E_UNSUPPORTED: pair activations (GEGLU / SimpleGate) need (Cout/2) % 32 == 0, got {half}")
        idx = torch.arange(cout, device=dev).view(2, half // 32, 32).permute(1, 0, 2).reshape(-1)
        wp = wp[idx]
        b = b[idx] if b is not None else None
        cout_out = half
    kcm = kh == 3 and (groups == 1 or (group_halo and cout_p == cout)) and cin_p % 64 == 0 and (c1 is None or c1 % 64 == 0)
    if kcm:
        wp = wp.reshape(cout_p, kh * kw, cin_p // 64, 64).permute(0, 2, 1, 3)
    return PackedConv(wp.reshape(cout_p, kh * kw * cin_p).to(_act).contiguous(),
                      None if b is None else b.contiguous(), cin_p, cout_p, cout_out, kh, groups, pair, kcm=kcm)


def _conv_desc(x, pc: PackedConv, x2, stride, pad, upsample, out_hw, plan_only) -> ConvDesc:
    n, h, w_, c1 = x.shape
    c2 = 0 if x2 is None else x2.shape[-1]
    k, g = pc.k, pc.groups
    if pad is None:
        pad = (k // 2, k // 2)
    if out_hw is None:
        hin, win = (h * 2, w_ * 2) if upsample else (h, w_)
        out_hw = ((hin + 2 * pad[0] - k) // stride + 1, (win + 2 * pad[1] - k) // stride + 1)
    d = ConvDesc()
    d.dtype = _dt(x)
    if plan_only:
        d.x, d.x2, d.w = 16, (16 if c2 else None), 16
    else:
        d.x, d.x2, d.w = _ptr(x), _ptr(x2), _ptr(pc.w)
    ws = workspace(x.device)
    d.workspace, d.workspace_bytes = ws.data_ptr(), ws.numel() * 4
    d.N, d.H, d.W = n, h, w_
    d.C1, d.ldx, d.C2, d.ldx2 = (c1 // g if g > 1 else c1), c1, c2, c2
    d.Cout, d.ldw, d.ldy = pc.cout // g, pc.w.shape[1], pc.cout_out
    d.KH = d.KW = k
    d.stride, d.pad_t, d.pad_l = stride, pad[0], pad[1]
    d.OH, d.OW = out_hw
    d.upsample2x, d.out_scale = int(upsample), 1.0
    d.k_chunk_major = int(pc.kcm and (c2 == 0 or c1 % 64 == 0))
    if wants_frag(pc, n, h, w_, c1, c2, stride, upsample, g) and pad == (1, 1):
        d.w_frag = 16 if plan_only else pc.frag().data_ptr()
    d.nbatch = g
    if g > 1:
        d.bs_x, d.bs_w, d.bs_bias, d.bs_y, d.bs_r = c1 // g, (pc.cout // g) * pc.w.shape[1], pc.cout // g, pc.cout_out // g, pc.cout_out // g
    return d


def conv(x: torch.Tensor, pc: PackedConv, *, x2=None, residual=None, bias=None, act=UR_ACT_NONE, stride=1, pad=None,
         out_hw=None, upsample=False, out_f32=False, out_scale=1.0, out=None, yt=None, n_split=0, t_rows=0,
         gn=False, store=True, rows=False, ln_stats=None, gn_ab=None, gn_silu=False):
    if x.dtype not in (BF16, F16) or x.dtype != pc.w.dtype or not x.is_contiguous() or x.dim() != 4:
        raise ValueError(f"conv: x must be a contiguous 4-d {pc.w.dtype} tensor, got {x.dtype} {tuple(x.shape)}")
    n, h, w_, c1 = x.shape
    c2 = 0 if x2 is None else x2.shape[-1]
    if (c1 + c2) != pc.cin * pc.groups:
        raise ValueError(f"conv: Cin mismatch: {c1}+{c2} vs {pc.cin}*{pc.groups}")
    d = _conv_desc(x, pc, x2, stride, pad, upsample, out_hw, plan_only=False)
    assert not pc.kcm or d.k_chunk_major, "chunk-major weights need a 64-aligned concat boundary"
    oh, ow = d.OH, d.OW
    co_total = pc.cout_out
    if out is None and store:
        out = torch.empty((n, oh, ow, co_total), dtype=torch.float32 if out_f32 else x.dtype, device=x.device)
    bias_t = pc.bias if bias is None else bias
    d.bias = _ptr(bias_t)
    if bias is not None and bias.dim() == 2 and bias.shape[0] > 1:
        d.bias_img_stride = bias.shape[1]
    d.residual, d.y, d.yt = _ptr(residual), _ptr(out), _ptr(yt)
    if ln_stats is not None:
        assert pc.ln_colsum is not None, "weights were not packed with pack_linear_ln"
        st, parts = ln_stats
        d.ln_stats, d.ln_colsum, d.ln_eps, d.ln_dim, d.ln_parts = st.data_ptr(), pc.ln_colsum.data_ptr(), pc.ln_eps, pc.cin, parts
    if gn_ab is not None:
        d.gn_ab, d.gn_silu = gn_ab.data_ptr(), int(gn_silu)
    if out is not None:
        d.ldy = out.shape[-1]
    d.ldr = residual.shape[-1] if residual is not None else 0
    d.act, d.out_f32, d.out_scale = act, int(out_f32), out_scale
    d.n_split, d.t_rows = n_split, t_rows
    d.t_ld = yt.shape[-1] if yt is not None else 0
    stats = rstats = None
    if gn or rows:
        if gn:
            d.gn_part = 16
        if rows:
            d.row_stats = 16
        plan = ConvPlan()
        check(lib.ur_conv2d_plan(d, plan))
        if gn:
            if not store and not plan.gn_fused:
                raise NotImplementedError("store=False needs a launch whose epilogue writes the statistics (conv_plan().gn_fused)")
            stats = (torch.empty((n, plan.gn_parts, co_total, 2), dtype=torch.float32, device=x.device), plan.gn_parts)
            d.gn_part = stats[0].data_ptr()
        if rows:
            rstats = (torch.empty((plan.row_stat_parts, n * oh * ow, 2), dtype=torch.float32, device=x.device), plan.row_stat_parts)
            d.row_stats = rstats[0].data_ptr()
    check(lib.ur_conv2d_nhwc(d, _stream()))
    if not store:
        return stats
    if stats is not None:
        out._gn = stats
    if rstats is not None:
        out._ln = rstats
    return out


def conv_plan(x: torch.Tensor, pc: PackedConv, *, x2=None, stride=1, pad=None, upsample=False, gn=False, gn_ab=False,
              act=UR_ACT_NONE, residual=False, store=True) -> ConvPlan:
    d = _conv_desc(x, pc, x2, stride, pad, upsample, None, plan_only=True)
    d.y = 16 if store else None
    d.residual = 16 if residual else None
    d.gn_part = 16 if gn else None
    d.gn_ab = 16 if gn_ab else None
    d.ldr = pc.cout_out if residual else 0
    d.act = act
    plan = ConvPlan()
    check(lib.ur_conv2d_plan(d, plan))
    return plan


def conv_launch(x: torch.Tensor, pc: PackedConv, *, x2=None, stride=1, pad=None, upsample=False, gn=False, gn_ab=False,
                act=UR_ACT_NONE, residual=False, store=True):
    d = _conv_desc(x, pc, x2, stride, pad, upsample, None, plan_only=True)
    d.y = 16 if store else None
    d.residual = 16 if residual else None
    d.gn_part = 16 if gn else None
    d.gn_ab = 16 if gn_ab else None
    d.ldr = pc.cout_out if residual else 0
    d.act = act
    return capi.plan_launch(d)


def pack_linear_ln(weight, bias, gamma, beta, eps, dev, *, pair=False) -> PackedConv:
    w = weight.detach().to(dev, torch.float32)
    g, b0 = gamma.detach().to(dev, torch.float32), beta.detach().to(dev, torch.float32)
    wf = w * g[None, :]
    t = w @ b0 + (bias.detach().to(dev, torch.float32) if bias is not None else 0.0)
    pc = pack_conv(wf, t, dev, pair=pair)
    pc.ln_colsum = pc.w.float().sum(dim=1).contiguous()
    pc.ln_eps = float(eps)
    return pc


def linear(x: torch.Tensor, pc: PackedConv, **kw):
    shp = x.shape
    rows = x.numel() // shp[-1]
    res = kw.pop("residual", None)
    if res is not None:
        res = res.reshape(1, 1, rows, res.shape[-1])
    gn = kw.pop("gn", False)
    gn_hw = kw.pop("gn_hw", None)
    if kw.get("ln_stats") is None and getattr(pc, "ln_colsum", None) is not None:
        raise ValueError("LayerNorm-folded weights need ln_stats")
    if gn:
        n_img, hw = gn_hw
        y = conv(x.reshape(n_img, 1, hw, shp[-1]), pc, residual=None if res is None else res.reshape(n_img, 1, hw, -1), gn=True, **kw)
    else:
        y = conv(x.reshape(1, 1, rows, shp[-1]), pc, residual=res, **kw)
    return None if y is None else carry(y, y.reshape(*shp[:-1], y.shape[-1]))


def bmm_nt(a: torch.Tensor, bmat: torch.Tensor, *, out_f32=False, out_scale=1.0):
    B, M, K = a.shape
    N = bmat.shape[1]
    if a.dtype != bmat.dtype or a.dtype not in (BF16, F16):
        raise ValueError(f"bmm_nt: both operands must share one 16-bit type, got {a.dtype} and {bmat.dtype}")
    assert a.stride(2) == 1 and bmat.stride(2) == 1 and K % 8 == 0 and N % 4 == 0
    out = torch.empty((B, M, N), dtype=torch.float32 if out_f32 else a.dtype, device=a.device)
    d = ConvDesc()
    d.dtype = _dt(a)
    d.x, d.w, d.y = a.data_ptr(), bmat.data_ptr(), out.data_ptr()
    ws = workspace(a.device)
    d.workspace, d.workspace_bytes = ws.data_ptr(), ws.numel() * 4
    d.N, d.H, d.W, d.C1, d.ldx, d.Cout, d.ldw, d.ldy = 1, 1, M, K, a.stride(1), N, bmat.stride(1), N
    d.KH = d.KW = 1
    d.stride, d.OH, d.OW, d.out_f32, d.out_scale, d.nbatch = 1, 1, M, int(out_f32), out_scale, B
    d.bs_x, d.bs_w, d.bs_y = a.stride(0), bmat.stride(0), M * N
    check(lib.ur_conv2d_nhwc(d, _stream()))
    return out


def gn_partials(x: torch.Tensor):
    pre = gn_of(x)
    if pre is not None:
        return pre
    n, c = x.shape[0], x.shape[-1]
    hw = x.numel() // (n * c)
    parts = lib.ur_groupnorm_stats_parts(n, hw, c)
    if parts <= 0:
        check(parts if parts < 0 else -1)
    plane = torch.empty((n, parts, c, 2), dtype=torch.float32, device=x.device)
    check(lib.ur_groupnorm_stats(x.data_ptr(), plane.data_ptr(), n, hw, c, _dt(x), _stream()))
    return plane, parts


def gn_finalize(x: torch.Tensor, gamma, beta, groups: int, eps: float, x2=None, use_pre=True, want_mean=False):
    n, c1 = x.shape[0], x.shape[-1]
    c2 = 0 if x2 is None else x2.shape[-1]
    hw = x.numel() // (n * c1)
    if not use_pre:
        x = x.view(x.shape)
        x2 = None if x2 is None else x2.view(x2.shape)
    p1, n1 = gn_partials(x)
    p2, n2 = gn_partials(x2) if x2 is not None else (None, 0)
    out = torch.empty((n, groups) if want_mean else (n, 2, c1 + c2), dtype=torch.float32, device=x.device)
    check(lib.ur_groupnorm_finalize(p1.data_ptr(), n1, c1, _ptr(p2), n2, c2, _ptr(gamma), _ptr(beta), n, hw, groups, eps,
                                    None if want_mean else out.data_ptr(), out.data_ptr() if want_mean else None, _stream()))
    return out


def gn_finalize_planes(plane: torch.Tensor, parts: int, hw: int):
    n, c = plane.shape[0], plane.shape[2]
    out = torch.empty((n, c), dtype=torch.float32, device=plane.device)
    check(lib.ur_groupnorm_finalize(plane.data_ptr(), parts, c, None, 0, 0, None, None, n, hw, c, 0.0, None, out.data_ptr(), _stream()))
    return out


def gn_apply(x: torch.Tensor, ab: torch.Tensor, silu=False, x2=None):
    n, c1 = x.shape[0], x.shape[-1]
    c2 = 0 if x2 is None else x2.shape[-1]
    hw = x.numel() // (n * c1)
    out = torch.empty((*x.shape[:-1], c1 + c2), dtype=x.dtype, device=x.device)
    check(lib.ur_groupnorm_apply_act(x.data_ptr(), _ptr(x2), out.data_ptr(), ab.data_ptr(), n, hw, c1, c2, int(silu), _dt(x), _stream()))
    return out


def group_norm(x: torch.Tensor, gamma, beta, groups: int, eps: float, silu=False, x2=None, use_pre=True):
    assert x.dtype in (BF16, F16) and x.is_contiguous()
    return gn_apply(x, gn_finalize(x, gamma, beta, groups, eps, x2=x2, use_pre=use_pre), silu, x2=x2)


def layer_norm(x: torch.Tensor, gamma, beta, eps: float):
    assert x.dtype in (BF16, F16) and x.is_contiguous()
    c = x.shape[-1]
    out = torch.empty_like(x)
    check(lib.ur_layernorm_rows(x.data_ptr(), out.data_ptr(), _ptr(gamma), _ptr(beta), x.numel() // c, c, eps, _dt(x), _stream()))
    return out


def softmax_rows(s: torch.Tensor, ldp=None):
    cols = s.shape[-1]
    ldp = ldp or round_up(cols, 8)
    p = torch.empty((*s.shape[:-1], ldp), dtype=_act, device=s.device)
    check(lib.ur_softmax_rows_f32(s.data_ptr(), p.data_ptr(), s.numel() // cols, cols, ldp, _dt(), _stream()))
    return p


def attention(q, k, vt, heads: int, head_dim: int, tq: int, tk: int, scale: float, *, ldq, ldk, bs_q, bs_k, bs_vt,
              batch: int, out=None):
    c = heads * head_dim
    if not (q.dtype == k.dtype == vt.dtype) or q.dtype not in (BF16, F16):
        raise ValueError(f"attention: q, k, v^T must share one 16-bit type, got {q.dtype}, {k.dtype}, {vt.dtype}")
    out = torch.empty((batch, tq, c), dtype=q.dtype, device=q.device) if out is None else out
    nws = lib.ur_attention_workspace_bytes(batch, heads, tq, tk, head_dim)
    ws = torch.empty(nws, dtype=torch.uint8, device=q.device) if nws else None
    check(lib.ur_attention_fwd_ws(q.data_ptr(), k.data_ptr(), vt.data_ptr(), out.data_ptr(), batch, heads, tq, tk, head_dim,
                                  ldq, ldk, vt.shape[-1], c, bs_q, bs_k, bs_vt, tq * c, scale, _ptr(ws), nws, _dt(q), _stream()))
    return out


def dwconv3x3(x, w9c, bias, gate=False):
    n, h, w_, c = x.shape
    out = torch.empty((n, h, w_, c // 2 if gate else c), dtype=x.dtype, device=x.device)
    check(lib.ur_dwconv3x3_nhwc(x.data_ptr(), w9c.data_ptr(), bias.data_ptr(), out.data_ptr(), n, h, w_, c, int(gate), _dt(x), _stream()))
    return out


def avgpool(x):
    return gn_finalize(x, None, None, x.shape[-1], 0.0, want_mean=True)


def scale_channels(x, s, residual=None):
    n, c = x.shape[0], x.shape[-1]
    out = torch.empty_like(x)
    check(lib.ur_scale_channels(x.data_ptr(), s.data_ptr(), _ptr(residual), out.data_ptr(), n, x.numel() // (n * c), c, _dt(x), _stream()))
    return out


FANOUT_MAX_K = 8


def scale_channels_fanout(x, s, k):
    b, c = x.shape[0], x.shape[-1]
    if s is not None and (s.dtype != torch.float32 or tuple(s.shape) != (k * b, c) or not s.is_contiguous()):
        raise ValueError(f"scale_channels_fanout: s must be a contiguous fp32 [{k * b}, {c}] tensor, got {s.dtype} {tuple(s.shape)}")
    if not x.is_contiguous():
        raise ValueError("scale_channels_fanout: x must be contiguous")
    out = torch.empty((k * b, *x.shape[1:]), dtype=x.dtype, device=x.device)
    for k0 in range(0, k, FANOUT_MAX_K):
        check(lib.ur_scale_channels_fanout(x.data_ptr(), None if s is None else s[k0 * b:].data_ptr(), out[k0 * b:].data_ptr(), b,
                                           min(FANOUT_MAX_K, k - k0), x.numel() // (b * c), c, _dt(x), _stream()))
    return out


def spade_modulate(n, gb, residual=None):
    c = n.shape[-1]
    out = torch.empty_like(n)
    check(lib.ur_spade_modulate(n.data_ptr(), gb.data_ptr(), gb.shape[-1], _ptr(residual), out.data_ptr(), n.numel() // c, c, _dt(n), _stream()))
    return out


def axpy_channels(a, b, s):
    c = a.shape[-1]
    out = torch.empty_like(a)
    check(lib.ur_axpy_channels(a.data_ptr(), b.data_ptr(), s.data_ptr(), out.data_ptr(), a.numel() // c, c, _dt(a), _stream()))
    return out


def linear_f32(x, w, bias, act=UR_ACT_NONE, groups=1):
    m, k = x.shape
    n = w.shape[0]
    out = torch.empty((m, n), dtype=torch.float32, device=x.device)
    check(lib.ur_linear_f32(x.data_ptr(), w.data_ptr(), _ptr(bias), out.data_ptr(), m, n, k, groups, act, _stream()))
    return out


def tfa_prompt_update(pooled, cond):
    b, t, d = cond.shape
    upd = torch.empty_like(cond)
    check(lib.ur_tfa_prompt_update(pooled.data_ptr(), cond.data_ptr(), upd.data_ptr(), b, t, d, _stream()))
    return upd


def tfa_prompt_update_fanout(pooled, cond, b, k, cond_per_row):
    rows, t, d = cond.shape
    if rows != (k * b if cond_per_row else k) or pooled.shape[0] != b or pooled.numel() != b * 3 * t * d:
        raise ValueError(f"tfa_prompt_update_fanout: pooled {tuple(pooled.shape)} / cond {tuple(cond.shape)} do not fit b={b}, k={k}")
    if not (pooled.is_contiguous() and cond.is_contiguous() and pooled.dtype == cond.dtype == torch.float32):
        raise ValueError("tfa_prompt_update_fanout: pooled and cond must be contiguous fp32 tensors")
    upd = torch.empty((k * b, t, d), dtype=torch.float32, device=cond.device)
    check(lib.ur_tfa_prompt_update_fanout(pooled.data_ptr(), cond.data_ptr(), upd.data_ptr(), b, k, t, d, int(bool(cond_per_row)), _stream()))
    return upd


def vec_mul_group(a, b, groups):
    out = torch.empty_like(a)
    check(lib.ur_vec_mul_group(a.data_ptr(), b.data_ptr(), out.data_ptr(), a.shape[0], a.shape[1], groups, _stream()))
    return out


def nchw_to_nhwc(x: torch.Tensor, cpad=None, image=False):
    x = x.contiguous().float()
    n, c, h, w_ = x.shape
    cpad = cpad or round_up(c, 8)
    out = torch.empty((n, h, w_, cpad), dtype=_act, device=x.device)
    fn = lib.ur_image_to_nhwc if image else lib.ur_nchw_f32_to_nhwc
    check(fn(x.data_ptr(), out.data_ptr(), n, c, h, w_, cpad, _dt(), _stream()))
    return out


def image_resize_pad(img: torch.Tensor, rh: int, rw: int, ph: int, pw: int, mul=2.0, add=-1.0, cpad=None):
    img = img.contiguous().float()
    n, c, h, w_ = img.shape
    cpad = cpad or round_up(c, 8)
    out = torch.empty((n, rh + ph, rw + pw, cpad), dtype=_act, device=img.device)
    check(lib.ur_image_resize_pad_nhwc(img.data_ptr(), out.data_ptr(), n, c, h, w_, rh, rw, ph, pw, cpad, mul, add, _dt(), _stream()))
    return out


def image_unpad_resize(x: torch.Tensor, c: int, crop_hw, out_hw, mul=1.0, add=0.0, quantize=False):
    n, xh, xw, ld = x.shape
    out = torch.empty((n, c, out_hw[0], out_hw[1]), dtype=torch.float32, device=x.device)
    check(lib.ur_image_unpad_resize_nchw(x.data_ptr(), int(x.dtype == torch.float32), out.data_ptr(), n, c, xh, xw, ld, crop_hw[0],
                                         crop_hw[1], out_hw[0], out_hw[1], mul, add, int(quantize), _dt() if x.dtype == torch.float32 else _dt(x), _stream()))
    return out


def ragged_geometry(sizes, canvas):
    ch, cw = int(canvas[0]), int(canvas[1])
    rows = []
    for n, row in enumerate(sizes):
        h, w, rh, rw = (int(v) for v in row)
        if not (0 < h <= rh <= ch and 0 < w <= rw <= cw and ch - rh < rh and cw - rw < rw):
            raise ValueError(f"ragged geometry: image {n} (H, W, RH, RW) = {(h, w, rh, rw)} does not fit the canvas {(ch, cw)}: "
                             "needs H <= RH <= CH, W <= RW <= CW and a reflect padding smaller than the resized image")
        rows.append((h, w, rh, rw))
# ... 526 lines not shown
```

Measured before the change: 30.61 images/s.

## Share first control-branch resnet head across denoise steps instead of repeating stem

The control encoder's first resnet block no longer runs on the stem repeated once per step. It runs norm1 and conv1 once on the un-repeated stem, and the per-step time-embedding bias is folded into a shifted GroupNorm finalize plus a broadcasting apply kernel. The residual add in conv2 reads the shared stem through a modulo row index. This removes nsteps-1 redundant copies of the first GN+conv1, at the cost of new kernels and a modulo in conv epilogue and prologue loads.

```diff
diff --git a/include/unirestore_hip.h b/include/unirestore_hip.h
--- a/include/unirestore_hip.h
+++ b/include/unirestore_hip.h
@@ -62,6 +62,7 @@
   long long bias_img_stride;
   int dtype;
   const void* w_frag;
+  int res_images;
 } ur_conv_desc;
 
 int ur_conv2d_nhwc(const ur_conv_desc* d, ur_stream_t stream);
@@ -102,6 +103,10 @@
                           const float* beta, int N, int HW, int G, float eps, float* ab, float* mean_out, ur_stream_t stream);
 int ur_groupnorm_apply_act(const void* x, const void* x2, void* y, const float* ab, int N, int HW, int C1, int C2, int silu,
                            int dtype, ur_stream_t stream);
+int ur_groupnorm_finalize_shifted(const float* part, int parts, const float* shift, int S, const float* gamma, const float* beta,
+                                  int B, int HW, int C, int G, float eps, float* ab, ur_stream_t stream);
+int ur_groupnorm_apply_act_bcast(const void* x, void* y, const float* ab, int rows, int src_images, int HW, int C, int silu, int dtype,
+                                 ur_stream_t stream);
 int ur_groupnorm_nhwc(const void* x, const void* x2, void* y, const float* gamma, const float* beta, int N, int HW,
                       int C1, int C2, int G, float eps, int silu, float* ws, float* ab, const float* pre1, int parts1,
                       const float* pre2, int parts2, int dtype, ur_stream_t stream);
diff --git a/unirestore_amd/capi.py b/unirestore_amd/capi.py
--- a/unirestore_amd/capi.py
+++ b/unirestore_amd/capi.py
@@ -29,7 +29,7 @@
         ("nbatch", C.c_int),
         ("bs_x", C.c_longlong), ("bs_x2", C.c_longlong), ("bs_w", C.c_longlong), ("bs_bias", C.c_longlong),
         ("bs_y", C.c_longlong), ("bs_r", C.c_longlong), ("k_chunk_major", C.c_int), ("bias_img_stride", C.c_longlong),
-        ("dtype", C.c_int), ("w_frag", C.c_void_p),
+        ("dtype", C.c_int), ("w_frag", C.c_void_p), ("res_images", C.c_int),
     ]
 
 
@@ -65,6 +65,8 @@
     "ur_instnorm_stats": (_I, [_P, _P, _I, _I, _I, _I, _P]),
     "ur_groupnorm_finalize": (_I, [_P, _I, _I, _P, _I, _I, _P, _P, _I, _I, _I, _F, _P, _P, _P]),
     "ur_groupnorm_apply_act": (_I, [_P, _P, _P, _P, _I, _I, _I, _I, _I, _I, _P]),
+    "ur_groupnorm_finalize_shifted": (_I, [_P, _I, _P, _I, _P, _P, _I, _I, _I, _I, _F, _P, _P]),
+    "ur_groupnorm_apply_act_bcast": (_I, [_P, _P, _P, _I, _I, _I, _I, _I, _I, _P]),
     "ur_groupnorm_nhwc": (_I, [_P, _P, _P, _P, _P, _I, _I, _I, _I, _I, _F, _I, _P, _P, _P, _I, _P, _I, _I, _P]),
     "ur_layernorm_rows": (_I, [_P, _P, _P, _P, _LL, _I, _F, _I, _P]),
     "ur_softmax_rows_f32": (_I, [_P, _P, _LL, _I, _I, _I, _P]),
diff --git a/unirestore_amd/csrc/igemm.hip b/unirestore_amd/csrc/igemm.hip
--- a/unirestore_amd/csrc/igemm.hip
+++ b/unirestore_amd/csrc/igemm.hip
@@ -106,6 +106,8 @@
   UR_REQUIRE(!d->y || (d->out_f32 ? d->ldy % 4 == 0 : d->ldy % 4 == 0), "ldy%4");
   UR_REQUIRE(!d->residual || d->ldr % 4 == 0, "ldr%4");
   UR_REQUIRE(!d->yt || (d->t_rows > 0 && d->n_split % 4 == 0 && !pair), "bad transposed-output spec");
+  UR_REQUIRE(d->res_images == 0 || (d->residual && d->res_images > 0 && d->res_images <= d->N && d->nbatch == 1),
+             "res_images needs a residual, 0 < res_images <= N and nbatch == 1");
 
   ConvK k;
   k.x = (const uint16_t*)d->x; k.x2 = (const uint16_t*)d->x2; k.w = (const uint16_t*)d->w; k.bias = d->bias;
@@ -115,6 +117,7 @@
   k.Cin = d->C1 + d->C2; k.Cout = d->Cout; k.ldw = d->ldw; k.ldy = d->ldy; k.ldr = d->ldr;
   k.KH = d->KH; k.KW = d->KW; k.stride = d->stride; k.pad_t = d->pad_t; k.pad_l = d->pad_l;
   k.OH = d->OH; k.OW = d->OW; k.OHW = d->OH * d->OW; k.ups = d->upsample2x; k.act = d->act; k.out_f32 = d->out_f32;
+  k.res_M = d->res_images && d->res_images < d->N ? d->res_images * d->OH * d->OW : 0;
   k.n_split = d->yt ? d->n_split : d->Cout; k.t_rows = d->t_rows; k.t_ld = d->t_ld;
   k.out_scale = d->out_scale;
   k.M = d->N * d->OH * d->OW; k.Ktot = d->KH * d->KW * k.Cin; k.nk = (k.Ktot + 63) / 64; k.nbatch = d->nbatch;
diff --git a/unirestore_amd/csrc/igemm_impl.h b/unirestore_amd/csrc/igemm_impl.h
--- a/unirestore_amd/csrc/igemm_impl.h
+++ b/unirestore_amd/csrc/igemm_impl.h
@@ -31,6 +31,7 @@
   int kcm;
   const uint16_t* wf;
   int wmajor;
+  int res_M;
   int xgm, xbn;
 };
 
@@ -73,7 +74,7 @@
 template <bool F16>
 __device__ __forceinline__ void epi_store(const ConvK& p, int gb, int m, int co, float v[4]) {
   if (p.res) {
-    const uint16_t* r = p.res + gb * p.bs_r + (long long)m * p.ldr + co;
+    const uint16_t* r = p.res + gb * p.bs_r + (long long)(p.res_M ? m % p.res_M : m) * p.ldr + co;
     uint2 rv = *reinterpret_cast<const uint2*>(r);
     v[0] += Act<F16>::lo(rv.x); v[1] += Act<F16>::hi(rv.x);
     v[2] += Act<F16>::lo(rv.y); v[3] += Act<F16>::hi(rv.y);
@@ -138,7 +139,9 @@
       const int r = i / Q, c = (i - r * Q) * 8;
       const int m = tile_row_to_m(p, m0, i < TOT ? r : 0);
       ok[u] = i < TOT && m < M && c < cmax;
-      gp[u] = g + (long long)(ok[u] ? m : m0) * ld + c0 + (ok[u] ? c : 0);
+      int mg = ok[u] ? m : m0;
+      if (LOAD && p.res_M) mg %= p.res_M;
+      gp[u] = g + (long long)mg * ld + c0 + (ok[u] ? c : 0);
       lp[u] = reinterpret_cast<uint2*>(smem + (ok[u] ? r * SROW + c * 2 : 0));
       if (LOAD) v[u] = *reinterpret_cast<const uint4*>(gp[u]);
       else { const uint2 a = lp[u][0], b = lp[u][1]; v[u] = make_uint4(a.x, a.y, b.x, b.y); }
@@ -730,7 +733,7 @@
         continue;
       }
       if (p.res) {
-        const uint2 rv = *reinterpret_cast<const uint2*>(p.res + (long long)m * p.ldr + co);
+        const uint2 rv = *reinterpret_cast<const uint2*>(p.res + (long long)(p.res_M ? m % p.res_M : m) * p.ldr + co);
         v[0] += Act<F16>::lo(rv.x); v[1] += Act<F16>::hi(rv.x);
         v[2] += Act<F16>::lo(rv.y); v[3] += Act<F16>::hi(rv.y);
       }
@@ -769,7 +772,7 @@
         const float4 t = *reinterpret_cast<const float4*>(p.ws + ((long long)sp * p.M + m) * p.Cout + co);
         v[i][0] += t.x; v[i][1] += t.y; v[i][2] += t.z; v[i][3] += t.w;
       }
-      rv[i] = p.res ? *reinterpret_cast<const uint2*>(p.res + (long long)m * p.ldr + co) : make_uint2(0, 0);
+      rv[i] = p.res ? *reinterpret_cast<const uint2*>(p.res + (long long)(p.res_M ? m % p.res_M : m) * p.ldr + co) : make_uint2(0, 0);
     }
     const float g[4] = {0, 0, 0, 0};
 #pragma unroll
diff --git a/unirestore_amd/csrc/norms.hip b/unirestore_amd/csrc/norms.hip
--- a/unirestore_amd/csrc/norms.hip
+++ b/unirestore_amd/csrc/norms.hip
@@ -92,16 +92,58 @@
     }
 }
 
+__global__ void gn_finalize_shifted_kernel(const float* __restrict__ p1, int P, int C, const float* __restrict__ shift, int B,
+                                           const float* __restrict__ gamma, const float* __restrict__ beta, int G, float eps,
+                                           double hw, double inv_cnt, float* __restrict__ ab) {
+  __shared__ double red[2][256];
+  const int g = blockIdx.x, r = blockIdx.y, t = threadIdx.x, NT = blockDim.x;
+  const int n = r % B;
+  const float* dsh = shift + (long long)(r / B) * C;
+  const int cpg = C / G, c_lo = g * cpg;
+  float ga0 = 1.f, be0 = 0.f, d0 = 0.f;
+  if (t < cpg) { ga0 = gamma ? gamma[c_lo + t] : 1.f; be0 = beta ? beta[c_lo + t] : 0.f; d0 = dsh[c_lo + t]; }
+  double s = 0.0, q = 0.0;
+  for (int idx = t; idx < cpg * P; idx += NT) {
+    const int p = idx / cpg, c = c_lo + (idx - p * cpg);
+    const float2 v = *reinterpret_cast<const float2*>(p1 + (((long long)n * P + p) * C + c) * 2);
+    const double d = (double)dsh[c];
+    s += (double)v.x; q += (double)v.y + 2.0 * d * (double)v.x;
+    if (p == 0) { s += hw * d; q += hw * d * d; }
+  }
+  if (NT == 64) {
+#pragma unroll
+    for (int o = 32; o > 0; o >>= 1) { s += __shfl_xor(s, o, 64); q += __shfl_xor(q, o, 64); }
+  } else {
+    red[0][t] = s; red[1][t] = q;
+    __syncthreads();
+    for (int o = NT >> 1; o > 0; o >>= 1) {
+      if (t < o) { red[0][t] += red[0][t + o]; red[1][t] += red[1][t + o]; }
+      __syncthreads();
+    }
+  }
+  const double S = NT == 64 ? s : red[0][0], Q = NT == 64 ? q : red[1][0];
+  const double mean = S * inv_cnt;
+  const double var = fma(Q, inv_cnt, -mean * mean);
+  const float rstd = rsqrtf(fmaxf((float)var, 0.f) + eps);
+  for (int i = t; i < cpg; i += NT) {
+    const int c = c_lo + i;
+    const float a = rstd * (i == t ? ga0 : (gamma ? gamma[c] : 1.f));
+    const float b = (i == t ? be0 : (beta ? beta[c] : 0.f)) - (float)mean * a;
+    ab[((long long)r * 2) * C + c] = a;
+    ab[((long long)r * 2 + 1) * C + c] = b + a * (i == t ? d0 : dsh[c]);
+  }
+}
+
 template <bool F16>
 __device__ __forceinline__ void gn_apply_body(const uint16_t* __restrict__ x, uint16_t* __restrict__ y,
                                               const float* __restrict__ ab, int HW, int C, int silu,
-                                              int pix_per_block, int c_off, int C_total, int CVS, int bx, int bz) {
+                                              int pix_per_block, int c_off, int C_total, int CVS, int bx, int bz, int xn) {
   const int n = blockIdx.y, t = threadIdx.x;
   const int CV = C >> 3, R = 256 / CVS;
   const int r = t / CVS, v = bz * CVS + (t - r * CVS);
   if (r >= R || v >= CV) return;
   const int p_begin = bx * pix_per_block, p_end = min(HW, p_begin + pix_per_block);
-  const uint16_t* xi = x + (long long)n * HW * C + v * 8;
+  const uint16_t* xi = x + (long long)xn * HW * C + v * 8;
   uint4 raw[4];
   if (p_begin + r < p_end) {
 #pragma unroll
@@ -139,16 +181,22 @@
 __global__ __launch_bounds__(256) void gn_apply_kernel(const uint16_t* __restrict__ x, uint16_t* __restrict__ y,
                                                        const float* __restrict__ ab, int HW, int C, int silu,
                                                        int pix_per_block, int c_off, int C_total, int CVS) {
-  gn_apply_body<F16>(x, y, ab, HW, C, silu, pix_per_block, c_off, C_total, CVS, blockIdx.x, blockIdx.z);
+  gn_apply_body<F16>(x, y, ab, HW, C, silu, pix_per_block, c_off, C_total, CVS, blockIdx.x, blockIdx.z, blockIdx.y);
+}
+template <bool F16>
+__global__ __launch_bounds__(256) void gn_apply_bcast_kernel(const uint16_t* __restrict__ x, uint16_t* __restrict__ y,
+                                                             const float* __restrict__ ab, int HW, int C, int silu,
+                                                             int pix_per_block, int CVS, int src_images) {
+  gn_apply_body<F16>(x, y, ab, HW, C, silu, pix_per_block, 0, C, CVS, blockIdx.x, blockIdx.z, (int)blockIdx.y % src_images);
 }
 template <bool F16>
 __global__ __launch_bounds__(256) void gn_apply2_kernel(const uint16_t* __restrict__ x1, const uint16_t* __restrict__ x2, uint16_t* __restrict__ y,
                                                         const float* __restrict__ ab, int HW, int C1, int C2, int silu, int ppb1, int ppb2,
                                                         int cvs1, int cvs2, int slabs1, int chunks1, int chunks2) {
   if ((int)blockIdx.z < slabs1) {
-    if ((int)blockIdx.x < chunks1) gn_apply_body<F16>(x1, y, ab, HW, C1, silu, ppb1, 0, C1 + C2, cvs1, blockIdx.x, blockIdx.z);
+    if ((int)blockIdx.x < chunks1) gn_apply_body<F16>(x1, y, ab, HW, C1, silu, ppb1, 0, C1 + C2, cvs1, blockIdx.x, blockIdx.z, blockIdx.y);
   } else if ((int)blockIdx.x < chunks2) {
-    gn_apply_body<F16>(x2, y, ab, HW, C2, silu, ppb2, C1, C1 + C2, cvs2, blockIdx.x, blockIdx.z - slabs1);
+    gn_apply_body<F16>(x2, y, ab, HW, C2, silu, ppb2, C1, C1 + C2, cvs2, blockIdx.x, blockIdx.z - slabs1, blockIdx.y);
   }
 }
 
@@ -333,6 +381,43 @@
   return ur::check_launch("ur_groupnorm_apply_act");
 }
 
+int ur_groupnorm_finalize_shifted(const float* part, int parts, const float* shift, int S, const float* gamma, const float* beta,
+                                  int B, int HW, int C, int G, float eps, float* ab, ur_stream_t stream) {
+  UR_REQUIRE(part && parts > 0 && shift && ab, "null pointer / no partials");
+  UR_REQUIRE(S > 0 && B > 0 && HW > 0 && C > 0 && G > 0 && C % G == 0, "bad args");
+  UR_REQUIRE((long long)S * B <= 65535, "S * B exceeds the grid");
+  hipStream_t s = (hipStream_t)stream;
+  const int cpg = C / G;
+  ur::ProfScope prof("groupnorm_finalize", 0.0, 8.0 * S * B * ((double)parts * C), s);
+  const int nt = (long long)cpg * parts <= 1024 ? 64 : 256;
+  hipLaunchKernelGGL(gn_finalize_shifted_kernel, dim3(G, S * B), dim3(nt), 0, s, part, parts, C, shift, B, gamma, beta, G, eps, (double)HW,
+                     1.0 / ((double)cpg * HW), ab);
+  return ur::check_launch("ur_groupnorm_finalize_shifted");
+}
+
+int ur_groupnorm_apply_act_bcast(const void* x, void* y, const float* ab, int rows, int src_images, int HW, int C, int silu, int dtype,
+                                 ur_stream_t stream) {
+  UR_REQUIRE(x && y && ab && rows > 0 && HW > 0, "null pointer / empty");
+  UR_REQUIRE_DT(dtype);
+  UR_REQUIRE(C > 0 && C % 8 == 0, "C must be a positive multiple of 8");
+  UR_REQUIRE(src_images > 0 && src_images <= rows && rows <= 65535, "0 < src_images <= rows <= 65535");
+  hipStream_t s = (hipStream_t)stream;
+  const char* fam = "groupnorm";
+  static const bool prof_shapes = getenv("UR_PROF_SHAPES") != nullptr;
+  if (prof_shapes) {
+    static std::map<std::string, int> interned;
+    char buf[96];
+    snprintf(buf, sizeof buf, "gn bcast N%d<-%d HW%d C%d", rows, src_images, HW, C);
+    fam = interned.emplace(buf, 0).first->first.c_str();
+  }
+  ur::ProfScope prof(fam, 0.0, 2.0 * ((double)rows + src_images) * HW * (double)C, s);
+  int cvs, slabs, chunks, ppb;
+  gn_geom(rows, HW, C, 2, cvs, slabs, chunks, ppb);
+  UR_DT_SWITCH(dtype, hipLaunchKernelGGL(gn_apply_bcast_kernel<F16>, dim3(chunks, rows, slabs), dim3(256), 0, s, (const uint16_t*)x, (uint16_t*)y, ab,
+                                         HW, C, silu, ppb, cvs, src_images));
+  return ur::check_launch("ur_groupnorm_apply_act_bcast");
+}
+
 int ur_groupnorm_nhwc(const void* x, const void* x2, void* y, const float* gamma, const float* beta, int N, int HW,
                       int C1, int C2, int G, float eps, int silu, float* ws, float* ab, const float* pre1, int parts1,
                       const float* pre2, int parts2, int dtype, ur_stream_t stream) {
diff --git a/unirestore_amd/csrc/runtime.hip b/unirestore_amd/csrc/runtime.hip
--- a/unirestore_amd/csrc/runtime.hip
+++ b/unirestore_amd/csrc/runtime.hip
@@ -75,7 +75,7 @@
 
 extern "C" {
 
-int ur_version(void) { return 101; }
+int ur_version(void) { return 102; }
 const char* ur_last_error(void) { return ur::g_err.c_str(); }
 
 int ur_profile_enable(int on) {
diff --git a/unirestore_amd/modules/model.py b/unirestore_amd/modules/model.py
--- a/unirestore_amd/modules/model.py
+++ b/unirestore_amd/modules/model.py
@@ -72,6 +72,9 @@
             chans.append(out)
         self.middle_block = MidBlock(out, temb, "self", head_dim=out // num_heads, groups=groups, eps=1e-5)
         self.fea_tran = nn.ModuleList([ResnetBlock2D(c, out_channels, temb, groups, 1e-5) for c in chans])
+        head = self.down_blocks[0].resnets[0]
+        assert head.conv_shortcut is None
+        head.shared_head = True
         for m in self.modules():
             if isinstance(m, ResnetBlock2D):
                 nn.init.zeros_(m.conv2.weight), nn.init.zeros_(m.conv2.bias)
@@ -87,12 +90,15 @@
     def stem(self, z_bf16):
         return ops.conv(z_bf16, self.conv_in.packed(), gn=True)
 
-    def run(self, stem, step):
+    def run(self, stem, step, shared=False):
         feats, h = [], stem
-        for blk in self.down_blocks:
+        for bi, blk in enumerate(self.down_blocks):
             states = []
             for i, res in enumerate(blk.resnets):
-                h = res.run(h, step=step)
+                if shared and bi == 0 and i == 0:
+                    h = res.run_shared(h, None if isinstance(step, str) else step)
+                else:
+                    h = res.run(h, step=step)
                 if blk.attn_kind == "self":
                     h = blk.attentions[i].run(h)
                 states.append(h)
@@ -105,20 +111,12 @@
 
     def run_schedule(self, stem, nsteps):
         b = stem.shape[0]
-        x = stem.repeat(nsteps, 1, 1, 1)
-        g = ops.gn_of(stem)
-        if g is not None:
-            x._gn = (g[0].repeat(nsteps, 1, 1, 1), g[1])
-        out = self.run(x, "all")
+        out = self.run(stem, "all", shared=True)
         return [{k: v[i * b:(i + 1) * b] for k, v in out.items()} for i in range(nsteps)]
 
     def run_steps(self, stem, s0, s1):
         b, n = stem.shape[0], s1 - s0
-        x = stem.repeat(n, 1, 1, 1)
-        g = ops.gn_of(stem)
-        if g is not None:
-            x._gn = (g[0].repeat(n, 1, 1, 1), g[1])
-        out = self.run(x, slice(s0, s1))
+        out = self.run(stem, slice(s0, s1), shared=True)
         return [{k: v[i * b:(i + 1) * b] for k, v in out.items()} for i in range(n)]
 
     def forward(self, x, timesteps, encoder_hidden_states=None):
diff --git a/unirestore_amd/modules/nn.py b/unirestore_amd/modules/nn.py
--- a/unirestore_amd/modules/nn.py
+++ b/unirestore_amd/modules/nn.py
@@ -106,6 +106,8 @@
         self.conv2 = Conv2d(cout, cout, 3, padding=1)
         self.conv_shortcut = Conv2d(cin, cout, 1) if cin != cout else None
         self.tbias = None
+        self.shared_head = False
+        self.tshift = None
 
     def set_time_table(self, silu_emb: torch.Tensor):
         for k in [k for k in self.__dict__ if isinstance(k, tuple) and k[:2] == ("cache", "tb_all")]:
@@ -113,6 +115,7 @@
         w, b = self.time_emb_proj.dev_f32()
         cb = self.conv1.bias.detach().float().to(DEV)
         self.tbias = ops.linear_f32(silu_emb, w, b + cb)
+        self.tshift = ops.linear_f32(silu_emb, w, b) if self.shared_head else None
 
     def _tbias_all(self, b, steps=None):
         key = ("cache", "tb_all", b) if steps is None else ("cache", "tb_all", b, steps.start, steps.stop)
@@ -144,6 +147,17 @@
             h = gn_silu_conv(self.norm2, h, pc2, gn=True)
             return self.spade.run(h, control[h.shape[2]], residual=sc)
         return gn_silu_conv(self.norm2, h, pc2, residual=sc, gn=True)
+
+
+    def run_shared(self, x, steps=None):
+        assert self.conv_shortcut is None and self.time_emb_proj is not None and "spade" not in self._modules
+        assert self.tshift is not None, "run_shared needs shared_head = True before set_time_table"
+        shift = self.tshift if steps is None else self.tshift[steps]
+        h0 = gn_silu_conv(self.norm1, x, self.conv1.packed(), gn=True)
+        g, b = self.norm2.dev()
+        ab = ops.gn_finalize_shifted(h0, shift, g, b, self.norm2.num_groups, self.norm2.eps)
+        h = ops.gn_apply_bcast(h0, ab, silu=True)
+        return ops.conv(h, self.conv2.packed(), residual=x, res_images=x.shape[0], gn=True)
 
 
 FUSE_GN_MIN_PIXELS = 256 * 256
diff --git a/unirestore_amd/ops.py b/unirestore_amd/ops.py
--- a/unirestore_amd/ops.py
+++ b/unirestore_amd/ops.py
@@ -171,7 +171,7 @@
 
 def conv(x: torch.Tensor, pc: PackedConv, *, x2=None, residual=None, bias=None, act=UR_ACT_NONE, stride=1, pad=None,
          out_hw=None, upsample=False, out_f32=False, out_scale=1.0, out=None, yt=None, n_split=0, t_rows=0,
-         gn=False, store=True, rows=False, ln_stats=None, gn_ab=None, gn_silu=False):
+         gn=False, store=True, rows=False, ln_stats=None, gn_ab=None, gn_silu=False, res_images=0):
     if x.dtype not in (BF16, F16) or x.dtype != pc.w.dtype or not x.is_contiguous() or x.dim() != 4:
         raise ValueError(f"conv: x must be a contiguous 4-d {pc.w.dtype} tensor, got {x.dtype} {tuple(x.shape)}")
     n, h, w_, c1 = x.shape
@@ -198,6 +198,10 @@
     if out is not None:
         d.ldy = out.shape[-1]
     d.ldr = residual.shape[-1] if residual is not None else 0
+    if res_images:
+        if residual is None or residual.shape[0] != res_images or not 0 < res_images <= n:
+            raise ValueError(f"conv: res_images={res_images} needs a residual of that many images (<= N={n})")
+        d.res_images = res_images
     d.act, d.out_f32, d.out_scale = act, int(out_f32), out_scale
     d.n_split, d.t_rows = n_split, t_rows
     d.t_ld = yt.shape[-1] if yt is not None else 0
@@ -344,6 +348,27 @@
     hw = x.numel() // (n * c1)
     out = torch.empty((*x.shape[:-1], c1 + c2), dtype=x.dtype, device=x.device)
     check(lib.ur_groupnorm_apply_act(x.data_ptr(), _ptr(x2), out.data_ptr(), ab.data_ptr(), n, hw, c1, c2, int(silu), _dt(x), _stream()))
+    return out
+
+
+def gn_finalize_shifted(x: torch.Tensor, shift: torch.Tensor, gamma, beta, groups: int, eps: float):
+    n, c = x.shape[0], x.shape[-1]
+    hw = x.numel() // (n * c)
+    if shift.dtype != torch.float32 or shift.dim() != 2 or shift.shape[1] != c or not shift.is_contiguous():
+        raise ValueError(f"gn_finalize_shifted: shift must be a contiguous fp32 [S, {c}] table, got {shift.dtype} {tuple(shift.shape)}")
+    plane, parts = gn_partials(x)
+    out = torch.empty((shift.shape[0] * n, 2, c), dtype=torch.float32, device=x.device)
+    check(lib.ur_groupnorm_finalize_shifted(plane.data_ptr(), parts, shift.data_ptr(), shift.shape[0], _ptr(gamma), _ptr(beta), n, hw, c,
+                                            groups, eps, out.data_ptr(), _stream()))
+    return out
+
+
+def gn_apply_bcast(x: torch.Tensor, ab: torch.Tensor, silu=False):
+    n, c = x.shape[0], x.shape[-1]
+    hw = x.numel() // (n * c)
+    rows = ab.shape[0]
+    out = torch.empty((rows, *x.shape[1:]), dtype=x.dtype, device=x.device)
+    check(lib.ur_groupnorm_apply_act_bcast(x.data_ptr(), out.data_ptr(), ab.data_ptr(), rows, n, hw, c, int(silu), _dt(x), _stream()))
     return out
 
 
```

New measurement: 30.67 images/s, median of 6. No clear change (+0.2%).
